# ur-whitelab/nmrgnn

Hardware: AMD Instinct MI355X
Metric: atoms/s (fwd+bwd) on 256-atom/16-neighbor synthetic graphs (higher is better)
Workload: dtype f32 (2xf16-piece MFMA, f32 accumulate)

## Files before the change

include/nmrgnn_hip.h:

```cpp
#ifndef NMRGNN_HIP_H
#define NMRGNN_HIP_H

#include <stdint.h>

#ifdef __cplusplus
extern "C" {
#endif

#define NG_ABI_VERSION 9

enum {
  NG_OK = 0,
  NG_ERR_INVALID = -1,
  NG_ERR_HIP = -2,
  NG_ERR_NOMEM = -3,
  NG_ERR_UNSUPPORTED = -4
};

enum { NG_ACT_NONE = 0, NG_ACT_SOFTPLUS = 1, NG_ACT_RELU = 2, NG_ACT_TANH = 3 };

typedef struct ng_ctx ng_ctx;

int ng_abi_version(void);
int ng_ctx_create(int device, ng_ctx** out);
void ng_ctx_destroy(ng_ctx* ctx);
const char* ng_last_error(ng_ctx* ctx);
int ng_reload_env(void);
int ng_weights_frozen(ng_ctx* ctx, int owner);
int ng_weights_changed(ng_ctx* ctx);
int ng_defer_reductions(ng_ctx* ctx, void* stream, int on);
int ng_flush_reductions(ng_ctx* ctx, void* stream);
int ng_ctx_set_graph_span(ng_ctx* ctx, int64_t max_graph_atoms);
int ng_ctx_reserve(ng_ctx* ctx, uint64_t bytes);

int ng_replay_arm(ng_ctx* ctx, int on);
int ng_replay_stage(ng_ctx* ctx, void* stream, uint64_t seed, float lr, float beta1, float beta2, int64_t step, int n_copies,
                    const void* const* src, void* const* dst, const uint64_t* bytes);
int ng_replay_token(ng_ctx* ctx, uint64_t* token);
int ng_replay_commit(ng_ctx* ctx, uint64_t token);

int ng_prof_enable(ng_ctx* ctx, int on);
int ng_prof_reset(ng_ctx* ctx);
int ng_prof_read(ng_ctx* ctx, int cap, const char** names, double* total_ms, int64_t* count);

int ng_randn(ng_ctx*, void* stream, uint64_t seed, uint64_t offset, float* out, int64_t n);
int ng_dropout_mask(ng_ctx*, void* stream, uint64_t seed, uint64_t offset, float keep, float* out,
                    int64_t n);

int ng_add_noise(ng_ctx*, void* stream, uint64_t seed, uint64_t offset, int64_t n, const float* x, float alpha,
                 float* out);
int ng_add_scaled(ng_ctx*, void* stream, int64_t n, const float* x, const float* y, float alpha,
                  float* out);

int ng_rbf_expand(ng_ctx*, void* stream, int64_t n, int H, const float* d_src, const float* d_eff,
                  const float* centers, float gap, float* out);

int ng_edge_mlp_fwd(ng_ctx*, void* stream, int64_t n_edges, int H, int E, int Le, int act,
                    const float* d_src, const float* d_eff, const float* centers, float gap,
                    const float* const* W, const float* const* b, float* e_out, float* z_save);
int ng_edge_tape_layout(int H, int E, int Le, int act, int64_t n_edges);
int ng_edge_mlp_bwd(ng_ctx*, void* stream, int64_t n_edges, int H, int E, int Le, int act,
                    const float* d_src, const float* d_eff, const float* centers, float gap,
                    const float* const* W, const float* z_save, const float* de,
                    float* const* dW, float* const* db);
int ng_edge_mlp_bwd_tape(ng_ctx*, void* stream, int64_t n_edges, int H, int E, int Le, int act,
                         const float* d_src, const float* d_eff, const float* centers, float gap,
                         const float* const* W, const float* z_save, const float* de,
                         float* const* dW, float* const* db, int tape_layout);

int ng_build_live_edges(ng_ctx*, void* stream, int64_t n_slots, const float* edges, int32_t* perm, int32_t* pos,
                        float* d_c, int32_t* n_live);
int ng_build_graph_lists(ng_ctx*, void* stream, int64_t N, int K, const int32_t* nlist, const float* edges, int32_t* nlist_c,
                         int32_t* csc_ptr, int32_t* csc_edge, int32_t* perm, int32_t* pos, float* d_c, int32_t* n_live);
int ng_graph_lists_one_launch(int64_t N, int K);
int ng_add_noise_live(ng_ctx*, void* stream, uint64_t seed, uint64_t offset, int64_t n, const float* x, const float* y,
                      float alpha, const int32_t* pos, float* out_c);
int ng_edge_live_supported(int H, int E, int Le, int act);
int ng_edge_mlp_fwd_live(ng_ctx*, void* stream, int64_t n_slots, int H, int E, int Le, int act,
                         const float* d_src_c, const float* d_eff_c, const int32_t* perm, const int32_t* n_live,
                         const float* centers, float gap, const float* const* W, const float* const* b,
                         float* e_out, float* z_save);
int ng_edge_mlp_bwd_live(ng_ctx*, void* stream, int64_t n_slots, int H, int E, int Le, int act,
                         const float* d_src_c, const float* d_eff_c, const int32_t* perm, const int32_t* n_live,
                         const float* centers, float gap, const float* const* W, const float* z_save,
                         const float* de, float* const* dW, float* const* db, int tape_layout);

int ng_edge_mlp_dinput(ng_ctx*, void* stream, int64_t n_slots, int H, int E, int Le, int act, const float* d_src,
                       const float* d_eff, const int32_t* perm, const int32_t* n_live, const float* centers, float gap,
                       const float* const* W, const float* const* b, const float* de, float* J_out, float* dd_out);
int ng_positions_grad(ng_ctx*, void* stream, int64_t N, int K, const float* pos, const int32_t* nlist, const float* edges,
                      const float* dd, float scale, const int32_t* csc_ptr, const int32_t* csc_edge, float* dpos);
int ng_positions_grad_csr(ng_ctx*, void* stream, int64_t N, int64_t nnz, const float* pos, const int32_t* row_ptr,
                          const int32_t* col, const int32_t* row_of, const float* dd, float scale, const int32_t* csc_ptr,
                          const int32_t* csc_edge, float* dpos);
int ng_positions_grad_pbc(ng_ctx*, void* stream, int64_t N, int K, const float* pos, const int32_t* nlist,
                          const float* edges, const float* dd, float scale, const int32_t* csc_ptr, const int32_t* csc_edge,
                          int n, const float* box, int triclinic, float* dpos);
int ng_positions_grad_csr_pbc(ng_ctx*, void* stream, int64_t N, int64_t nnz, const float* pos, const int32_t* row_ptr,
                              const int32_t* col, const int32_t* row_of, const float* dd, float scale,
                              const int32_t* csc_ptr, const int32_t* csc_edge, int n, const float* box, int triclinic,
                              float* dpos);
int ng_box_grad(ng_ctx*, void* stream, int64_t N, int K, const float* pos, const int32_t* nlist, const float* edges,
                const float* dd, float scale, int G, const int32_t* graph_ptr, const float* box, int triclinic, double* strain,
                double* dvec);
int ng_box_grad_csr(ng_ctx*, void* stream, int64_t N, int64_t nnz, const float* pos, const int32_t* row_ptr,
                    const int32_t* col, const float* dd, float scale, int G, const int32_t* graph_ptr, const float* box,
                    int triclinic, double* strain, double* dvec);
int ng_positions_grad_ragged_pbc(ng_ctx*, void* stream, int64_t N, int K, const float* pos, const int32_t* nlist,
                                 const float* edges, const float* dd, float scale, const int32_t* csc_ptr,
                                 const int32_t* csc_edge, int G, const int32_t* graph_ptr, const float* box,
                                 const int32_t* kind, const int32_t* kind_host, float* dpos);
int ng_positions_grad_csr_ragged_pbc(ng_ctx*, void* stream, int64_t N, int64_t nnz, const float* pos, const int32_t* row_ptr,
                                     const int32_t* col, const int32_t* row_of, const float* dd, float scale,
                                     const int32_t* csc_ptr, const int32_t* csc_edge, int G, const int32_t* graph_ptr,
                                     const float* box, const int32_t* kind, const int32_t* kind_host, float* dpos);
int ng_box_grad_ragged(ng_ctx*, void* stream, int64_t N, int K, const float* pos, const int32_t* nlist, const float* edges,
                       const float* dd, float scale, int G, const int32_t* graph_ptr, const float* box, const int32_t* kind,
                       const int32_t* kind_host, double* strain, double* dvec);
int ng_box_grad_csr_ragged(ng_ctx*, void* stream, int64_t N, int64_t nnz, const float* pos, const int32_t* row_ptr,
                           const int32_t* col, const float* dd, float scale, int G, const int32_t* graph_ptr,
                           const float* box, const int32_t* kind, const int32_t* kind_host, double* strain, double* dvec);

int ng_embed_fwd(ng_ctx*, void* stream, int64_t N, int C, int F, const float* atoms,
                 const float* Wemb, float* h0);
int ng_embed_bwd(ng_ctx*, void* stream, int64_t N, int C, int F, const float* atoms,
                 const float* dh0, float* dWemb);

int ng_mp_aggregate(ng_ctx*, void* stream, int64_t N, int K, int F, int E, const float* h,
                    const int32_t* nlist, const float* e, float* A);

int ng_mp_layer_fwd(ng_ctx*, void* stream, int64_t N, int K, int F, int E, int act, int residual,
                    const float* h, const int32_t* nlist, const float* e, const float* inv_degree,
                    const float* w, float* h_out, float* A_save, float* s_save);
int ng_mp_layer_wants_aggregate(int F, int E, int K);

int ng_mp_layer_bwd(ng_ctx*, void* stream, int64_t N, int K, int F, int E, int act,
                    const float* h, const int32_t* nlist, const float* e, const float* inv_degree,
                    const float* w, const float* A_save, const float* s_save,
                    const int32_t* csc_ptr, const int32_t* csc_edge, const float* dh_out,
                    float* dh_in, float* de, int de_accum, float* dw);

int ng_mp_edge_records(ng_ctx*, void* stream, int64_t N, int K, int E, const int32_t* csc_ptr,
                       const int32_t* csc_edge, const float* e, float* rec);
int ng_mp_layer_bwd_rec(ng_ctx*, void* stream, int64_t N, int K, int F, int E, int act,
                    const float* h, const int32_t* nlist, const float* e, const float* inv_degree,
                    const float* w, const float* A_save, const float* s_save,
                    const int32_t* csc_ptr, const int32_t* csc_edge, const float* dh_out,
                    float* dh_in, float* de, int de_accum, float* dw, const float* csc_rec);

int ng_mp_aggregate_csr(ng_ctx*, void* stream, int64_t N, int F, int E, const float* h,
                        const int32_t* row_ptr, const int32_t* col, const float* e, float* A);
int ng_mp_layer_fwd_csr(ng_ctx*, void* stream, int64_t N, int64_t nnz, int F, int E, int act, int residual,
                        const float* h, const int32_t* row_ptr, const int32_t* col, const float* e,
                        const float* inv_degree, const float* w, float* h_out, float* A_save, float* s_save);
int ng_mp_layer_bwd_csr(ng_ctx*, void* stream, int64_t N, int64_t nnz, int F, int E, int act, const float* h,
                        const int32_t* row_ptr, const int32_t* col, const int32_t* row_of, const float* e,
                        const float* inv_degree, const float* w, const float* A_save, const float* s_save,
                        const int32_t* csc_ptr, const int32_t* csc_edge, const float* dh_out, float* dh_in,
                        float* de, int de_accum, float* dw);

int ng_mp_layer_fwd_short(ng_ctx*, void* stream, int64_t N, int K, int F, int E, int act, int residual, const float* h,
                          const int32_t* nlist, const float* e, const float* inv_degree, const float* w, float* h_out);
int ng_mp_layer_fwd_short_csr(ng_ctx*, void* stream, int64_t N, int F, int E, int act, int residual, const float* h,
                              const int32_t* row_ptr, const int32_t* col, const float* e, const float* inv_degree,
                              const float* w, float* h_out);
int ng_mp_layer_short_ok(int64_t N, int K, int F, int E);
int ng_fc_head_ok(int64_t N, int F, int L, int C, int act);
int ng_fc_head_fwd(ng_ctx*, void* stream, int64_t N, int F, int L, int C, int act, const float* x,
                   const float* const* W, const float* const* b, const float* Wout, const float* bout,
                   const float* atoms, const float* pstd, const float* pavg, float* peaks);

int ng_build_incoming_lists(ng_ctx*, void* stream, int64_t N, int K, int64_t n_entries, const int32_t* nlist,
                            const float* edges, int32_t* nlist_c, int32_t* csc_ptr, int32_t* csc_edge);
size_t ng_incoming_lists_scratch_bytes(int64_t N, int64_t n_entries);

int ng_cutoff_count(ng_ctx*, void* stream, int G, int n, float cutoff, const float* pos, int32_t* deg);
int ng_cutoff_fill(ng_ctx*, void* stream, int G, int n, float cutoff, float scale, const float* pos,
                   const int32_t* row_ptr, int32_t* col, float* dist, float* inv_degree);
int ng_cutoff_fill_rows(ng_ctx*, void* stream, int G, int n, float cutoff, float scale, const float* pos,
                        const int32_t* row_ptr, int32_t* col, float* dist, float* inv_degree, int32_t* row_of);
int ng_cutoff_count_pbc(ng_ctx*, void* stream, int G, int n, float cutoff, const float* pos, const float* box, int triclinic,
                        int32_t* deg);
int ng_cutoff_fill_rows_pbc(ng_ctx*, void* stream, int G, int n, float cutoff, float scale, const float* pos,
                            const float* box, int triclinic, const int32_t* row_ptr, int32_t* col, float* dist,
                            float* inv_degree, int32_t* row_of);
int ng_exclusive_scan_i32(ng_ctx*, void* stream, int64_t n, const int32_t* in, int32_t* out);

int ng_knn_graph(ng_ctx*, void* stream, int G, int n, int K, float scale, const float* pos,
                 int32_t* nlist, float* edges, float* inv_degree);
int ng_knn_graph_pbc(ng_ctx*, void* stream, int G, int n, int K, float scale, const float* pos, const float* box,
                     int triclinic, int32_t* nlist, float* edges, float* inv_degree);
int ng_knn_graph_ragged(ng_ctx*, void* stream, int G, int64_t N, int K, float scale, const float* pos, const int32_t* graph_ptr,
                        const int32_t* graph_ptr_host, int max_n, int32_t* nlist, float* edges, float* inv_degree);
int ng_cutoff_count_ragged(ng_ctx*, void* stream, int G, int64_t N, float cutoff, const float* pos, const int32_t* graph_ptr,
                           int max_n, int32_t* deg);
int ng_cutoff_fill_rows_ragged(ng_ctx*, void* stream, int G, int64_t N, float cutoff, float scale, const float* pos,
                               const int32_t* graph_ptr, int max_n, const int32_t* row_ptr, int32_t* col, float* dist,
                               float* inv_degree, int32_t* row_of);
int ng_knn_graph_ragged_pbc(ng_ctx*, void* stream, int G, int64_t N, int K, float scale, const float* pos,
                            const int32_t* graph_ptr, const int32_t* graph_ptr_host, int max_n, const float* box,
                            const int32_t* kind, const int32_t* kind_host, int32_t* nlist, float* edges, float* inv_degree);
int ng_cutoff_count_ragged_pbc(ng_ctx*, void* stream, int G, int64_t N, float cutoff, const float* pos,
                               const int32_t* graph_ptr, int max_n, const float* box, const int32_t* kind,
                               const int32_t* kind_host, int32_t* deg);
int ng_cutoff_fill_rows_ragged_pbc(ng_ctx*, void* stream, int G, int64_t N, float cutoff, float scale, const float* pos,
                                   const int32_t* graph_ptr, int max_n, const float* box, const int32_t* kind,
                                   const int32_t* kind_host, const int32_t* row_ptr, int32_t* col, float* dist,
                                   float* inv_degree, int32_t* row_of);

int ng_amp_attend(ng_ctx*, void* stream, int64_t N, int K, int F, int E, const float* h,
                  const int32_t* nlist, const float* e, const float* inv_degree, const float* wq,
                  const float* wk, float* agg);
int ng_amp_attend_bwd(ng_ctx*, void* stream, int64_t N, int K, int F, int E, const float* h,
                      const int32_t* nlist, const float* e, const float* inv_degree, const float* wq,
                      const float* wk, const int32_t* in_ptr, const int32_t* in_slot, const float* dagg,
                      float* dh, float* de, float* dwq, float* dwk);

int ng_fc_block_fwd(ng_ctx*, void* stream, int64_t N, int F, int L, int act, const float* x,
                    const float* const* W, const float* const* b, float* const* y, float* g);

int64_t ng_fc_block_scratch_floats(int64_t N, int F, int L);
int ng_fc_block_bwd(ng_ctx*, void* stream, int64_t N, int F, int L, int act, const float* const* x,
                    const float* g, const float* const* W, const float* dg, float* dx, float* const* dW,
                    float* const* db, float* scratch);

int ng_dense_fwd(ng_ctx*, void* stream, int64_t M, int Kin, int Nout, int act, int residual,
                 const float* X, const float* W, const float* b, float* Y, float* s_save);
int ng_dense_bwd(ng_ctx*, void* stream, int64_t M, int Kin, int Nout, int act, int residual,
                 const float* X, const float* W, const float* s_save, const float* dY, float* dX,
                 float* dW, float* db);

// ... 64 lines not shown
```

nmrgnn_amd/_lib.py:

```python
from __future__ import annotations

import ctypes as C
import os
import threading

_HERE = os.path.dirname(os.path.abspath(__file__))
LIB_PATH = os.environ.get("NMRGNN_HIP_LIB") or os.path.join(_HERE, "csrc", "libnmrgnn_hip.so")

NG_ACT_NONE, NG_ACT_SOFTPLUS, NG_ACT_RELU, NG_ACT_TANH = 0, 1, 2, 3
ACT_CODES = {None: NG_ACT_NONE, "linear": NG_ACT_NONE, "softplus": NG_ACT_SOFTPLUS, "relu": NG_ACT_RELU,
             "tanh": NG_ACT_TANH}

_c_float_p = C.POINTER(C.c_float)
_c_int32_p = C.POINTER(C.c_int32)
_vp = C.c_void_p
_i64 = C.c_int64
_u64 = C.c_uint64
_int = C.c_int
_f = C.c_float

SIGNATURES = {
    "ng_abi_version": (_int, []),
    "ng_ctx_create": (_int, [_int, C.POINTER(_vp)]),
    "ng_ctx_destroy": (None, [_vp]),
    "ng_last_error": (C.c_char_p, [_vp]),
    "ng_ctx_reserve": (_int, [_vp, _u64]),
    "ng_replay_arm": (_int, [_vp, _int]),
    "ng_replay_stage": (_int, [_vp, _vp, _u64, _f, _f, _f, _i64, _int, C.POINTER(_vp), C.POINTER(_vp), C.POINTER(_u64)]),
    "ng_replay_token": (_int, [_vp, C.POINTER(_u64)]),
    "ng_replay_commit": (_int, [_vp, _u64]),
    "ng_reload_env": (_int, []),
    "ng_weights_frozen": (_int, [_vp, _int]),
    "ng_weights_changed": (_int, [_vp]),
    "ng_defer_reductions": (_int, [_vp, _vp, _int]),
    "ng_flush_reductions": (_int, [_vp, _vp]),
    "ng_ctx_set_graph_span": (_int, [_vp, _i64]),
    "ng_prof_enable": (_int, [_vp, _int]),
    "ng_prof_reset": (_int, [_vp]),
    "ng_prof_read": (_int, [_vp, _int, C.POINTER(C.c_char_p), C.POINTER(C.c_double), C.POINTER(_i64)]),
    "ng_randn": (_int, [_vp, _vp, _u64, _u64, _vp, _i64]),
    "ng_dropout_mask": (_int, [_vp, _vp, _u64, _u64, _f, _vp, _i64]),
    "ng_add_scaled": (_int, [_vp, _vp, _i64, _vp, _vp, _f, _vp]),
    "ng_add_noise": (_int, [_vp, _vp, _u64, _u64, _i64, _vp, _f, _vp]),
    "ng_rbf_expand": (_int, [_vp, _vp, _i64, _int, _vp, _vp, _vp, _f, _vp]),
    "ng_edge_mlp_fwd": (_int, [_vp, _vp, _i64, _int, _int, _int, _int, _vp, _vp, _vp, _f,
                               C.POINTER(_vp), C.POINTER(_vp), _vp, _vp]),
    "ng_edge_tape_layout": (_int, [_int, _int, _int, _int, _i64]),
    "ng_edge_table_range": (_int, [_vp, _vp, _i64, _int, _vp, _vp, _vp, _vp, _f, _vp]),
    "ng_edge_table_points": (_int, [_vp, _vp, _int, _int, _vp, _vp, _vp, _vp]),
    "ng_edge_table_check": (_int, [_vp, _vp, _int, _int, _vp, _f, _vp, _vp, _vp, _int, _vp, _vp]),
    "ng_edge_table_interp": (_int, [_vp, _vp, _i64, _int, _int, _vp, _vp, _vp, _vp, _vp, _vp, _vp]),
    "ng_edge_table_scatter": (_int, [_vp, _vp, _i64, _int, _int, _int, _vp, _vp, _vp, _vp, _vp, _vp]),
    "ng_edge_table_dinput": (_int, [_vp, _vp, _i64, _int, _int, _vp, _vp, _vp, _vp, _vp, _vp, _vp, _vp]),
    "ng_edge_mlp_bwd": (_int, [_vp, _vp, _i64, _int, _int, _int, _int, _vp, _vp, _vp, _f,
                               C.POINTER(_vp), _vp, _vp, C.POINTER(_vp), C.POINTER(_vp)]),
    "ng_edge_mlp_bwd_tape": (_int, [_vp, _vp, _i64, _int, _int, _int, _int, _vp, _vp, _vp, _f,
                                    C.POINTER(_vp), _vp, _vp, C.POINTER(_vp), C.POINTER(_vp), _int]),
    "ng_build_live_edges": (_int, [_vp, _vp, _i64, _vp, _vp, _vp, _vp, _vp]),
    "ng_build_graph_lists": (_int, [_vp, _vp, _i64, _int, _vp, _vp, _vp, _vp, _vp, _vp, _vp, _vp, _vp]),
    "ng_graph_lists_one_launch": (_int, [_i64, _int]),
    "ng_add_noise_live": (_int, [_vp, _vp, _u64, _u64, _i64, _vp, _vp, _f, _vp, _vp]),
    "ng_edge_live_supported": (_int, [_int, _int, _int, _int]),
    "ng_edge_mlp_fwd_live": (_int, [_vp, _vp, _i64, _int, _int, _int, _int, _vp, _vp, _vp, _vp, _vp, _f,
                                    C.POINTER(_vp), C.POINTER(_vp), _vp, _vp]),
    "ng_edge_mlp_bwd_live": (_int, [_vp, _vp, _i64, _int, _int, _int, _int, _vp, _vp, _vp, _vp, _vp, _f,
                                    C.POINTER(_vp), _vp, _vp, C.POINTER(_vp), C.POINTER(_vp), _int]),
    "ng_edge_mlp_dinput": (_int, [_vp, _vp, _i64, _int, _int, _int, _int, _vp, _vp, _vp, _vp, _vp, _f,
                                  C.POINTER(_vp), C.POINTER(_vp), _vp, _vp, _vp]),
    "ng_positions_grad": (_int, [_vp, _vp, _i64, _int, _vp, _vp, _vp, _vp, _f, _vp, _vp, _vp]),
    "ng_positions_grad_csr": (_int, [_vp, _vp, _i64, _i64, _vp, _vp, _vp, _vp, _vp, _f, _vp, _vp, _vp]),
    "ng_positions_grad_pbc": (_int, [_vp, _vp, _i64, _int, _vp, _vp, _vp, _vp, _f, _vp, _vp, _int, _vp, _int, _vp]),
    "ng_positions_grad_csr_pbc": (_int, [_vp, _vp, _i64, _i64, _vp, _vp, _vp, _vp, _vp, _f, _vp, _vp, _int, _vp, _int, _vp]),
    "ng_box_grad": (_int, [_vp, _vp, _i64, _int, _vp, _vp, _vp, _vp, _f, _int, _vp, _vp, _int, _vp, _vp]),
    "ng_box_grad_csr": (_int, [_vp, _vp, _i64, _i64, _vp, _vp, _vp, _vp, _f, _int, _vp, _vp, _int, _vp, _vp]),
    "ng_positions_grad_ragged_pbc": (_int, [_vp, _vp, _i64, _int, _vp, _vp, _vp, _vp, _f, _vp, _vp, _int, _vp, _vp, _vp, _vp, _vp]),
    "ng_positions_grad_csr_ragged_pbc": (_int, [_vp, _vp, _i64, _i64, _vp, _vp, _vp, _vp, _vp, _f, _vp, _vp, _int, _vp, _vp, _vp,
                                                _vp, _vp]),
    "ng_box_grad_ragged": (_int, [_vp, _vp, _i64, _int, _vp, _vp, _vp, _vp, _f, _int, _vp, _vp, _vp, _vp, _vp, _vp]),
    "ng_box_grad_csr_ragged": (_int, [_vp, _vp, _i64, _i64, _vp, _vp, _vp, _vp, _f, _int, _vp, _vp, _vp, _vp, _vp, _vp]),
    "ng_restraint_loss": (_int, [_vp, _vp, _int, _i64, _vp, _vp, _vp, _vp, _vp]),
    "ng_restraint_loss_ex": (_int, [_vp, _vp, _int, _i64, _int, _vp, _vp, _vp, _vp, _vp, _f, _vp, _vp, _vp, _vp]),
    "ng_embed_fwd": (_int, [_vp, _vp, _i64, _int, _int, _vp, _vp, _vp]),
    "ng_embed_bwd": (_int, [_vp, _vp, _i64, _int, _int, _vp, _vp, _vp]),
    "ng_mp_aggregate": (_int, [_vp, _vp, _i64, _int, _int, _int, _vp, _vp, _vp, _vp]),
    "ng_mp_layer_fwd": (_int, [_vp, _vp, _i64, _int, _int, _int, _int, _int, _vp, _vp, _vp, _vp, _vp,
                               _vp, _vp, _vp]),
    "ng_mp_layer_bwd": (_int, [_vp, _vp, _i64, _int, _int, _int, _int, _vp, _vp, _vp, _vp, _vp,
                               _vp, _vp, _vp, _vp, _vp, _vp, _vp, _int, _vp]),
    "ng_mp_layer_bwd_rec": (_int, [_vp, _vp, _i64, _int, _int, _int, _int, _vp, _vp, _vp, _vp, _vp,
                               _vp, _vp, _vp, _vp, _vp, _vp, _vp, _int, _vp, _vp]),
    "ng_mp_edge_records": (_int, [_vp, _vp, _i64, _int, _int, _vp, _vp, _vp, _vp]),
    "ng_mp_aggregate_csr": (_int, [_vp, _vp, _i64, _int, _int, _vp, _vp, _vp, _vp, _vp]),
    "ng_mp_layer_fwd_csr": (_int, [_vp, _vp, _i64, _i64, _int, _int, _int, _int, _vp, _vp, _vp, _vp, _vp, _vp,
                                   _vp, _vp, _vp]),
    "ng_mp_layer_bwd_csr": (_int, [_vp, _vp, _i64, _i64, _int, _int, _int, _vp, _vp, _vp, _vp, _vp, _vp, _vp,
                                   _vp, _vp, _vp, _vp, _vp, _vp, _vp, _int, _vp]),
    "ng_build_incoming_lists": (_int, [_vp, _vp, _i64, _int, _i64, _vp, _vp, _vp, _vp, _vp]),
    "ng_incoming_lists_scratch_bytes": (C.c_size_t, [_i64, _i64]),
    "ng_cutoff_count": (_int, [_vp, _vp, _int, _int, _f, _vp, _vp]),
    "ng_cutoff_fill": (_int, [_vp, _vp, _int, _int, _f, _f, _vp, _vp, _vp, _vp, _vp]),
    "ng_cutoff_fill_rows": (_int, [_vp, _vp, _int, _int, _f, _f, _vp, _vp, _vp, _vp, _vp, _vp]),
    "ng_cutoff_count_pbc": (_int, [_vp, _vp, _int, _int, _f, _vp, _vp, _int, _vp]),
    "ng_cutoff_fill_rows_pbc": (_int, [_vp, _vp, _int, _int, _f, _f, _vp, _vp, _int, _vp, _vp, _vp, _vp, _vp]),
    "ng_exclusive_scan_i32": (_int, [_vp, _vp, _i64, _vp, _vp]),
    "ng_dense_fwd": (_int, [_vp, _vp, _i64, _int, _int, _int, _int, _vp, _vp, _vp, _vp, _vp]),
    "ng_dense_bwd": (_int, [_vp, _vp, _i64, _int, _int, _int, _int, _vp, _vp, _vp, _vp, _vp, _vp,
                            _vp]),
    "ng_head_fwd": (_int, [_vp, _vp, _i64, _int, _int, _vp, _vp, _vp, _vp, _vp, _vp, _vp, _vp]),
    "ng_head_fwd_dropout": (_int, [_vp, _vp, _i64, _int, _int, _vp, _u64, _u64, _f, _vp, _vp, _vp, _vp, _vp, _vp, _vp]),
    "ng_head_bwd": (_int, [_vp, _vp, _i64, _int, _int, _vp, _vp, _vp, _vp, _vp, _vp, _vp, _vp, _vp]),
    "ng_head_loss_blocks": (_int, [_vp, _int, _int, _int, _i64]),
    "ng_head_loss_bwd": (_int, [_vp, _vp, _i64, _int, _int, _int, _i64, _vp, _u64, _u64, _f, _vp, _vp, _vp, _vp, _vp, _vp, _vp,
                               _vp, _vp, _f, _vp, _vp, _vp]),
    "ng_head_loss_reduce": (_int, [_vp, _vp, _vp, _int, _int, _int, _vp, _vp, _vp]),
    "ng_mp_layer_wants_aggregate": (_int, [_int, _int, _int]),
    "ng_fc_block_fwd": (_int, [_vp, _vp, _i64, _int, _int, _int, _vp, _vp, _vp, _vp, _vp]),
    "ng_fc_block_scratch_floats": (_i64, [_i64, _int, _int]),
    "ng_fc_block_bwd": (_int, [_vp, _vp, _i64, _int, _int, _int, _vp, _vp, _vp, _vp, _vp, _vp, _vp, _vp]),
    "ng_mp_layer_fwd_short": (_int, [_vp, _vp, _i64, _int, _int, _int, _int, _int, _vp, _vp, _vp, _vp, _vp, _vp]),
    "ng_mp_layer_fwd_short_csr": (_int, [_vp, _vp, _i64, _int, _int, _int, _int, _vp, _vp, _vp, _vp, _vp, _vp, _vp]),
    "ng_mp_layer_short_ok": (_int, [_i64, _int, _int, _int]),
    "ng_fc_head_ok": (_int, [_i64, _int, _int, _int, _int]),
    "ng_fc_head_fwd": (_int, [_vp, _vp, _i64, _int, _int, _int, _int, _vp, C.POINTER(_vp), C.POINTER(_vp), _vp, _vp, _vp,
                              _vp, _vp, _vp]),
    "ng_knn_graph": (_int, [_vp, _vp, _int, _int, _int, _f, _vp, _vp, _vp, _vp]),
    "ng_knn_graph_pbc": (_int, [_vp, _vp, _int, _int, _int, _f, _vp, _vp, _int, _vp, _vp, _vp]),
    "ng_knn_graph_ragged": (_int, [_vp, _vp, _int, _i64, _int, _f, _vp, _vp, _vp, _int, _vp, _vp, _vp]),
    "ng_cutoff_count_ragged": (_int, [_vp, _vp, _int, _i64, _f, _vp, _vp, _int, _vp]),
    "ng_cutoff_fill_rows_ragged": (_int, [_vp, _vp, _int, _i64, _f, _f, _vp, _vp, _int, _vp, _vp, _vp, _vp, _vp]),
    "ng_knn_graph_ragged_pbc": (_int, [_vp, _vp, _int, _i64, _int, _f, _vp, _vp, _vp, _int, _vp, _vp, _vp, _vp, _vp, _vp]),
    "ng_cutoff_count_ragged_pbc": (_int, [_vp, _vp, _int, _i64, _f, _vp, _vp, _int, _vp, _vp, _vp, _vp]),
    "ng_cutoff_fill_rows_ragged_pbc": (_int, [_vp, _vp, _int, _i64, _f, _f, _vp, _vp, _int, _vp, _vp, _vp, _vp, _vp, _vp, _vp,
                                              _vp]),
    "ng_amp_attend": (_int, [_vp, _vp, _i64, _int, _int, _int, _vp, _vp, _vp, _vp, _vp, _vp, _vp]),
    "ng_amp_attend_bwd": (_int, [_vp, _vp, _i64, _int, _int, _int] + [_vp] * 13),
    "ng_loss_l2": (_int, [_vp, _vp, _i64, _int, _vp, _vp, _vp, _vp, _vp, _vp]),
    "ng_loss_name": (_int, [_vp, _vp, _i64, _int, _vp, _vp, _vp, _vp, _f, _vp, _vp]),
    "ng_name_metrics": (_int, [_vp, _vp, _i64, _vp, _vp, _vp, _vp, _int, _vp, _int, _int, _vp]),
    "ng_adam_step": (_int, [_vp, _vp, _i64, _vp, _vp, _vp, _vp, _f, _f, _f, _f, _i64, _f]),
    "ng_comm_unique_id": (_int, [_vp]),
    "ng_comm_init": (_int, [_vp, _int, _int, _vp]),
    "ng_comm_destroy": (_int, [_vp]),
    "ng_comm_world": (_int, [_vp]),
    "ng_allreduce_grads": (_int, [_vp, _vp, _vp, _i64]),
}

_lib = None
_lock = threading.Lock()


class NGError(RuntimeError):
    pass


def load():
    global _lib
    with _lock:
        if _lib is not None:
            return _lib
        if not os.path.exists(LIB_PATH):
            raise NGError(
                f"{LIB_PATH} is missing — build it with `python -c 'import __graft_entry__ as g; "
                f"g.build()'` or `make -C nmrgnn_amd/csrc`. nmrgnn_amd has no CPU fallback.")
        lib = C.CDLL(LIB_PATH)
        for name, (res, args) in SIGNATURES.items():
            fn = getattr(lib, name)
            fn.restype = res
            fn.argtypes = args
        if lib.ng_abi_version() != 9:
            raise NGError("libnmrgnn_hip.so ABI version mismatch")
        _lib = lib
        return lib

# ... 73 lines not shown
```

nmrgnn_amd/csrc/edge_bwd_h2.hip:

```cpp
#include "edge_bwd_h2.cuh"

namespace ng {

template <bool LIVE>
__global__ __launch_bounds__(HX_THREADS, 1) void edge_bwd_h2_kernel(EdgeBwdH2Args a) {
  extern __shared__ __attribute__((aligned(16))) char smem_hx[];
  float* sWo4 = reinterpret_cast<float*>(smem_hx + HX_IMGS);
  float* sdE = sWo4 + FH * 4;
  float* sCen = sdE + FTM * 4;

  const int tid = threadIdx.x, lane = tid & 63, half = lane >> 5, l31 = lane & 31;
  const int wave = __builtin_amdgcn_readfirstlane(tid >> 6);
  const int kslab = wave >> 1, nsl0 = 2 * (wave & 1);
  const int zk = wave & 3, zrt = wave >> 2;
  const int cn = tid & 127, rq = tid >> 7;
  const int row = 32 * zrt + l31;
  const int col0 = 32 * zk + 4 * half;
  const int prz = hx_prow_z(row), prg = hx_prow_g(row);
  const int E = a.E;
  if (LIVE && __builtin_amdgcn_readfirstlane(*a.n_live) < 0) return;
  float gscale, ginv;
  {
    float* sred = reinterpret_cast<float*>(smem_hx);
    float m = 0.f;
// ... 236 lines not shown
    for (int r = 0; r < 16; ++r) chk += fabsf(accB[r]);
#pragma unroll
    for (int n = 0; n < 4; ++n) chk += fabsf(accWo[n]) + fabsf(accbo[n]);
    range_guard_raise(a.guard, not_finite(chk * ginv));
  }
  {
    const int k = kslab * 32 + l31;
#pragma unroll
    for (int l = 0; l < 3; ++l)
#pragma unroll
      for (int j = 0; j < 2; ++j)
#pragma unroll
        for (int q = 0; q < 4; ++q) {
          const int n = (nsl0 + j) * 32 + 8 * q + 4 * half;
          *reinterpret_cast<float4*>(part + l * FH * FH + k * FH + n) =
              make_float4(ginv * accW[l][j][4 * q + 0], ginv * accW[l][j][4 * q + 1], ginv * accW[l][j][4 * q + 2],
                          ginv * accW[l][j][4 * q + 3]);
        }
  }
  float* red = reinterpret_cast<float*>(smem_hx);
  float* dbw = reinterpret_cast<float*>(smem_hx + 2 * HX_IMG_Z);
  const int red_stride = 3 * FH + FH * E + E;
  {
    const int c = l31 / 5;
    if (c < 6 && l31 == 5 * c && (c & 1) >= 0) {
      const int layer = c >> 1, j = c & 1;
#pragma unroll
      for (int r = 0; r < 16; ++r)
        dbw[(kslab * 3 + layer) * FH + 32 * (nsl0 + j) + (r & 3) + 8 * (r >> 2) + 4 * half] = ginv * accB[r];
    }
  }
  if (zk == 0 && half == 0) *reinterpret_cast<float4*>(sdE + 4 * row) = make_float4(accbo[0], accbo[1], accbo[2], accbo[3]);
  __syncthreads();
#pragma unroll
  for (int l = 0; l < 3; ++l) red[rq * red_stride + l * FH + cn] = dbw[(rq * 3 + l) * FH + cn];
  for (int n = 0; n < E; ++n) red[rq * red_stride + 3 * FH + cn * E + n] = ginv * accWo[n];
  if (cn < E) {
    float sbo = 0.f;
    if (rq == 0)
      for (int r = 0; r < FTM; ++r) sbo += sdE[4 * r + cn];
    red[rq * red_stride + 3 * FH + FH * E + cn] = ginv * sbo;
  }
  __syncthreads();
  for (int t = tid; t < red_stride; t += HX_THREADS)
    part[3 * FH * FH + t] = red[t] + red[red_stride + t] + red[2 * red_stride + t] + red[3 * red_stride + t];
}

constexpr int HX_SCALE_BLOCKS = 1024;
constexpr int64_t HX_DIRECT_MAX = 32768;
__global__ __launch_bounds__(256) void hx_absmax_kernel(const float* __restrict__ de, int64_t n, float* __restrict__ blockmax,
                                                        const int32_t* __restrict__ n_live) {
  __shared__ float red[4];
  if (n_live && *n_live < 0) return;
  float m = 0.f;
  const int64_t n4 = (reinterpret_cast<uintptr_t>(de) & 15) == 0 ? n >> 2 : 0;
  const float4* de4 = reinterpret_cast<const float4*>(de);
  for (int64_t i = (int64_t)blockIdx.x * 256 + threadIdx.x; i < n4; i += (int64_t)gridDim.x * 256) {
    const float4 v = de4[i];
    m = fmaxf(fmaxf(m, fmaxf(fabsf(v.x), fabsf(v.y))), fmaxf(fabsf(v.z), fabsf(v.w)));
  }
  for (int64_t i = 4 * n4 + (int64_t)blockIdx.x * 256 + threadIdx.x; i < n; i += (int64_t)gridDim.x * 256) m = fmaxf(m, fabsf(de[i]));
#pragma unroll
  for (int o = 32; o > 0; o >>= 1) m = fmaxf(m, __shfl_xor(m, o));
  if ((threadIdx.x & 63) == 0) red[threadIdx.x >> 6] = m;
  __syncthreads();
  if (threadIdx.x == 0) blockmax[blockIdx.x] = fmaxf(fmaxf(red[0], red[1]), fmaxf(red[2], red[3]));
}

constexpr int64_t HX_SEG_EDGES = ((int64_t)1 << 23) - 256;
int edge_bwd_h2_segments(int64_t n_edges) { return (int)std::max<int64_t>(1, cdiv(n_edges, HX_SEG_EDGES)); }

bool edge_bwd_h2_supported(int E, int64_t n_edges) { (void)n_edges; return E >= 1 && E <= 4; }

bool edge_tape_blocked(int E, int64_t n_edges) {
  return edge_split_enabled() && !sw().edge_bwd_math_fp32 && edge_bwd_h2_supported(E, n_edges);
}
constexpr size_t HX_WT_BYTES = (size_t)2 * 4 * 8 * 2 * 1024;

size_t edge_bwd_h2_ws_bytes() { return HX_WT_BYTES + 16 + (size_t)(HX_SCALE_BLOCKS + 2) * 4; }

int edge_bwd_h2_launch(ng_ctx* ctx, hipStream_t st, int64_t n_edges, int E, const float* d_src, const float* d_eff,
                       const float* centers, float gap, const float* const* W, const float* z_save, const float* de,
                       char* wt_img, float* partial, int part_stride, int grid, int tape_blocked, RangeGuard guard,
                       LiveEdges live) {
  float* blockmax = reinterpret_cast<float*>(wt_img + HX_WT_BYTES + 16);
  int nb_max = 0;
  bool have_wt = false;
  char* wimg = (char*)cached_image(ctx, W[1], 13, HX_WT_BYTES + 16, &have_wt);
  const bool cached_wt = wimg != nullptr;
  if (!wimg) wimg = wt_img;
  {
    ProfScope ps(ctx, st, "edge_bwd_h2_prep");
    if (!have_wt) {
      PackJob j;
      j.kind = PK_EDGE_WT; j.blocks = 17; j.src[0] = W[1]; j.src[1] = W[2]; j.src[2] = W[3]; j.i0 = E; j.dst[0] = wimg;
      if (int rc = pack_launch(ctx, st, j)) return rc;
      if (cached_wt) cache_set_job(ctx, W[1], 13, j);
    }
    if (n_edges * E <= HX_DIRECT_MAX && (reinterpret_cast<uintptr_t>(de) & 15) == 0) {
      nb_max = -(int)(n_edges * E);
      blockmax = const_cast<float*>(de);
    } else {
      nb_max = (int)std::min<int64_t>(HX_SCALE_BLOCKS, cdiv(n_edges * E, 1024));
      hipLaunchKernelGGL(hx_absmax_kernel, dim3(nb_max), dim3(256), 0, st, de, n_edges * E, blockmax, live.n_live);
      NG_HIP(ctx, hipGetLastError());
    }
  }
  const int nseg = edge_bwd_h2_segments(n_edges);
  for (int sg = 0; sg < nseg; ++sg) {
    const int64_t e0 = (int64_t)sg * HX_SEG_EDGES;
    EdgeBwdH2Args a;
    a.n_edges = std::min<int64_t>(HX_SEG_EDGES, n_edges - e0); a.d_src = d_src + e0; a.d_eff = d_eff + e0; a.centers = centers;
    a.neg_inv_gap_log2e = (float)(-1.4426950408889634 / (double)gap);
    a.wt_img = wimg; a.blockmax = blockmax; a.n_blockmax = nb_max; a.Wo = W[3]; a.z_save = z_save + e0 * FH; a.z_layer_stride = n_edges * FH;
    a.de = live.perm ? de : de + e0 * E;
    a.perm = live.perm ? live.perm + e0 : nullptr; a.n_live = live.n_live; a.row_base = e0;
    a.partial = partial + (size_t)sg * grid * part_stride; a.part_stride = part_stride; a.E = E; a.tape_blocked = tape_blocked;
    a.guard = guard;
    ProfScope ps(ctx, st, "edge_bwd_h2");
    if (live.perm)
      hipLaunchKernelGGL(edge_bwd_h2_kernel<true>, dim3(grid), dim3(HX_THREADS), HX_LDS_BYTES, st, a);
    else
      hipLaunchKernelGGL(edge_bwd_h2_kernel<false>, dim3(grid), dim3(HX_THREADS), HX_LDS_BYTES, st, a);
    NG_HIP(ctx, hipGetLastError());
    if (sg + 1 < nseg) continue;
  }
  return NG_OK;
}

}
```

nmrgnn_amd/csrc/edge_fused.h:

```cpp
#pragma once
#include "ng_internal.h"

namespace ng {

constexpr int FH = 128;
constexpr int FTM = 64;
constexpr int FLD = FH + 4;
constexpr int FMAX_E = 8;

int edge_fused_pack(ng_ctx* ctx, hipStream_t st, const float* const* W, float* Wpk, float* WpkT);
PackJob edge_fused_pack_job(const float* const* W, float* Wpk, float* WpkT);

}

namespace ng {
int edge_fused_bwd(ng_ctx* ctx, hipStream_t st, int64_t n_edges, int E, const float* d_src,
                   const float* d_eff, const float* centers, float gap, const float* const* W,
                   const float* z_save, const float* de, float* const* dW, float* const* db, int tape_layout = -1,
                   LiveEdges live = LiveEdges());
}

#define NG_LDS_BARRIER()                                   \
  do {                                                     \
    asm volatile("s_waitcnt lgkmcnt(0)" ::: "memory");     \
    __builtin_amdgcn_s_barrier();                          \
    asm volatile("" ::: "memory");                         \
  } while (0)

namespace ng {
bool edge_split_enabled();
int edge_h2_fwd(ng_ctx* ctx, hipStream_t st, int64_t n_edges, int E, const float* d_src, const float* d_eff,
                const float* centers, float gap, const float* const* W, const float* const* b, float* e_out,
                float* z_save, LiveEdges live = LiveEdges());
bool edge_bwd_h2_supported(int E, int64_t n_edges);
int edge_bwd_h2_segments(int64_t n_edges);
bool edge_tape_blocked(int E, int64_t n_edges);
size_t edge_bwd_h2_ws_bytes();
int edge_bwd_h2_launch(ng_ctx* ctx, hipStream_t st, int64_t n_edges, int E, const float* d_src, const float* d_eff,
                       const float* centers, float gap, const float* const* W, const float* z_save, const float* de,
                       char* wt_img, float* partial, int part_stride, int grid, int tape_blocked, RangeGuard guard,
                       LiveEdges live = LiveEdges());
}
```

nmrgnn_amd/csrc/edge_fused_bwd.hip:

```cpp
#include <algorithm>

#include "mfma_gemm.cuh"
#include "edge_fused.h"

namespace ng {

constexpr int BW_THREADS = 512;

struct EdgeBwdArgs {
  int64_t n_edges;
  const float* d_src;
  const float* d_eff;
  const float* centers;
  float neg_inv_gap;
  const float* WpkT;
  const float* Wo;
  const float* z_save;
  const float* de;
  float* partial;
  int part_stride;
  int tape_blocked;
  int zero_rows;
  RangeGuard guard;
  const int32_t* perm;
// ... 209 lines not shown
      o.z = g[2] * (1.0f - __expf(-z.z));
      o.w = g[3] * (1.0f - __expf(-z.w));
      *reinterpret_cast<float4*>(bufC + row * FLD + c4 * 4) = o;
    }
#pragma unroll 4
    for (int r = 16 * rq; r < 16 * rq + 16; ++r) {
      const float z = bufA[r * FLD + cn];
#pragma unroll
      for (int n = 0; n < E; ++n) accWo[n] += z * sdE[r * E + n];
      if (cn < E) accbo += sdE[r * E + cn];
    }
    regs_to_lds(pzB, bufB, tid);
    NG_LDS_BARRIER();
    dw_gemm(accW[2], bufB, bufC, kslab, nsl0, lane);
    colsum16(accb[2], bufC, cn, rq);
    dz_gemm_epilogue(bufC, bufB, bufA, a.WpkT, 2, zk, zrt, lane);
    NG_LDS_BARRIER();
    regs_to_lds(pzA, bufC, tid);
    NG_LDS_BARRIER();
    dw_gemm(accW[1], bufC, bufA, kslab, nsl0, lane);
    colsum16(accb[1], bufA, cn, rq);
    dz_gemm_epilogue(bufA, bufC, bufB, a.WpkT, 1, zk, zrt, lane);
    NG_LDS_BARRIER();
#pragma unroll
    for (int i = 0; i < 4; ++i) {
      const int lin = tid + i * BW_THREADS;
      const int row = lin >> 5, c4 = lin & 31;
      const float d = sD[row], m = sM[row];
      const float4 mu = *reinterpret_cast<const float4*>(sCen + c4 * 4);
      const float u0 = d - mu.x, u1 = d - mu.y, u2 = d - mu.z, u3 = d - mu.w;
      float4 o;
      o.x = m * __expf(u0 * u0 * a.neg_inv_gap);
      o.y = m * __expf(u1 * u1 * a.neg_inv_gap);
      o.z = m * __expf(u2 * u2 * a.neg_inv_gap);
      o.w = m * __expf(u3 * u3 * a.neg_inv_gap);
      *reinterpret_cast<float4*>(bufA + row * FLD + c4 * 4) = o;
    }
    NG_LDS_BARRIER();
    if (tile + gridDim.x < ntiles) prefetch((tile + gridDim.x) * FTM);
    dw_gemm(accW[0], bufA, bufB, kslab, nsl0, lane);
    colsum16(accb[0], bufB, cn, rq);
    NG_LDS_BARRIER();
  }

  float* part = a.partial + (int64_t)blockIdx.x * a.part_stride;
  {
    const int half = lane >> 5, l31 = lane & 31;
    const int k = kslab * 32 + l31;
#pragma unroll
    for (int l = 0; l < 3; ++l)
#pragma unroll
      for (int j = 0; j < 2; ++j)
#pragma unroll
        for (int q = 0; q < 4; ++q) {
          const int n = (nsl0 + j) * 32 + 8 * q + 4 * half;
          *reinterpret_cast<float4*>(part + l * FH * FH + k * FH + n) =
              make_float4(accW[l][j][4 * q + 0], accW[l][j][4 * q + 1], accW[l][j][4 * q + 2],
                          accW[l][j][4 * q + 3]);
        }
  }
  float* red = bufA;
  const int red_stride = 3 * FH + FH * E + E;
#pragma unroll
  for (int l = 0; l < 3; ++l) red[rq * red_stride + l * FH + cn] = accb[l];
#pragma unroll
  for (int n = 0; n < E; ++n) red[rq * red_stride + 3 * FH + cn * E + n] = accWo[n];
  if (cn < E) red[rq * red_stride + 3 * FH + FH * E + cn] = accbo;
  __syncthreads();
  for (int t = tid; t < red_stride; t += BW_THREADS)
    part[3 * FH * FH + t] = red[t] + red[red_stride + t] + red[2 * red_stride + t] + red[3 * red_stride + t];
  for (int64_t rowz = (int64_t)gridDim.x + blockIdx.x; rowz < a.zero_rows; rowz += gridDim.x)
    for (int t = tid; t < a.part_stride; t += BW_THREADS) a.partial[rowz * a.part_stride + t] = 0.f;
}

struct BwdOut {
  float* dW[3];
  float* db[3];
  float* dWo;
  float* dbo;
};

__global__ __launch_bounds__(1024) void edge_bwd_reduce_kernel(const float* __restrict__ partial, int n_wg,
                                                               int stride, int E, BwdOut o, const int32_t* __restrict__ n_live) {
  __shared__ float red[16][64];
  const int total = bwd_part_floats(E);
  const int lane = threadIdx.x & 63, wv = threadIdx.x >> 6;
  const int idx = blockIdx.x * 64 + lane;
  float s = 0.f;
  if (n_live && *n_live < 0) n_wg = 0;
  if (idx < total) {
    const float* p = partial + idx;
    int w = wv;
    for (; w + 112 < n_wg; w += 128) {
      float v[8];
#pragma unroll
      for (int u = 0; u < 8; ++u) v[u] = p[(int64_t)(w + 16 * u) * stride];
#pragma unroll
      for (int u = 0; u < 8; ++u) s += v[u];
    }
    for (; w < n_wg; w += 16) s += p[(int64_t)w * stride];
  }
  red[wv][lane] = s;
  __syncthreads();
  if (wv != 0 || idx >= total) return;
  s = red[0][lane];
#pragma unroll
  for (int j = 1; j < 16; ++j) s += red[j][lane];
  int r = idx;
  if (r < 3 * FH * FH) { o.dW[r / (FH * FH)][r % (FH * FH)] = s; return; }
  r -= 3 * FH * FH;
  if (r < 3 * FH) { o.db[r / FH][r % FH] = s; return; }
  r -= 3 * FH;
  if (r < FH * E) { o.dWo[r] = s; return; }
  r -= FH * E;
  o.dbo[r] = s;
}

int edge_fused_bwd(ng_ctx* ctx, hipStream_t st, int64_t n_edges, int E, const float* d_src,
                   const float* d_eff, const float* centers, float gap, const float* const* W,
                   const float* z_save, const float* de, float* const* dW, float* const* db, int tape_layout,
                   LiveEdges live) {
  const int64_t ntiles = cdiv(n_edges, FTM);
  const int grid = (int)std::min<int64_t>(ntiles, (int64_t)ctx->num_cu);
  const int stride = (bwd_part_floats(E) + 3) / 4 * 4;
  const size_t pk_floats = (size_t)3 * FH * FH;
  const int nseg = edge_bwd_h2_segments(n_edges);
  bool haveT = false;
  float* WpkT = (float*)cached_image(ctx, W[0], 12, pk_floats * 4, &haveT);
  const bool cachedT = WpkT != nullptr;
  float* ws = (float*)workspace(ctx, (pk_floats + (size_t)nseg * grid * stride) * 4 + edge_bwd_h2_ws_bytes());
  if (!ws) return NG_ERR_NOMEM;
  if (!cachedT) WpkT = ws;
  float* partial = ws + pk_floats;
  if (!haveT) {
    const PackJob j = edge_fused_pack_job(W, nullptr, WpkT);
    if (int rc = pack_launch(ctx, st, j)) return rc;
    if (cachedT) cache_set_job(ctx, W[0], 12, j);
  }
  EdgeBwdArgs a;
  a.n_edges = n_edges; a.d_src = d_src; a.d_eff = d_eff; a.centers = centers;
  a.neg_inv_gap = (float)(-1.0 / (double)gap);
  a.WpkT = WpkT; a.Wo = W[3]; a.z_save = z_save; a.de = de;
  a.partial = partial; a.part_stride = stride;
  a.tape_blocked = 0; a.zero_rows = 0; a.guard = RangeGuard{nullptr, 0};
  a.perm = live.perm; a.n_live = live.n_live; a.z_layer_stride = n_edges * FH;
  const size_t lds = (size_t)(3 * FTM * FLD + FH * FMAX_E + FTM * FMAX_E + 2 * FTM + FH) * 4;
  const bool blocked = tape_layout < 0 ? edge_tape_blocked(E, n_edges) : tape_layout == 1;
  if (blocked && !edge_bwd_h2_supported(E, n_edges)) return fail(ctx, NG_ERR_INVALID, "edge_mlp_bwd: blocked tape for an unsupported shape");
  int n_part = grid;
  const bool split = blocked || edge_tape_blocked(E, n_edges);
  if (split) {
    const RangeGuard guard = range_guard_begin(ctx);
    if (!guard.word) return NG_ERR_NOMEM;
    int rc3 = edge_bwd_h2_launch(ctx, st, n_edges, E, d_src, d_eff, centers, gap, W, z_save, de,
                     (char*)(partial + (size_t)nseg * grid * stride), partial, stride, grid, blocked ? 1 : 0, guard, live);
    if (rc3) return rc3;
    n_part = nseg * grid;
    a.tape_blocked = blocked ? 1 : 0; a.zero_rows = n_part; a.guard = guard;
  }
  {
    ProfScope ps(ctx, st, split ? "edge_bwd_range_fallback" : "edge_fused_bwd");
#define NG_BW(EE)                                                                                   \
  case EE:                                                                                          \
    hipLaunchKernelGGL((edge_fused_bwd_kernel<EE>), dim3(grid), dim3(BW_THREADS), lds, st, a);      \
    break;
    switch (E) { NG_BW(1) NG_BW(2) NG_BW(3) NG_BW(4) NG_BW(5) NG_BW(6) NG_BW(7) NG_BW(8) }
#undef NG_BW
    NG_HIP(ctx, hipGetLastError());
  }
  {
    ProfScope ps(ctx, st, "edge_bwd_reduce");
    BwdOut o;
    for (int l = 0; l < 3; ++l) { o.dW[l] = dW[l]; o.db[l] = db[l]; }
    o.dWo = dW[3]; o.dbo = db[3];
    hipLaunchKernelGGL(edge_bwd_reduce_kernel, dim3((unsigned)cdiv(bwd_part_floats(E), 64)), dim3(1024), 0, st,
                       partial, n_part, stride, E, o, live.n_live);
    NG_HIP(ctx, hipGetLastError());
  }
  return NG_OK;
}

}
```

nmrgnn_amd/csrc/edge_ops.hip:

```cpp
#include <algorithm>

#include "mfma_gemm.cuh"
#include "edge_fused.h"

namespace ng {

constexpr int MAX_E = 8;

__global__ void rbf_kernel(int64_t n_edges, int H, const float* __restrict__ d_src,
                           const float* __restrict__ d_eff, const float* __restrict__ centers,
                           float neg_inv_gap, float* __restrict__ X0) {
  const int c4n = H / 4;
  const int64_t total = n_edges * c4n;
  for (int64_t t = (int64_t)blockIdx.x * blockDim.x + threadIdx.x; t < total;
       t += (int64_t)gridDim.x * blockDim.x) {
    const int64_t eidx = t / c4n;
    const int c4 = (int)(t % c4n);
    float4 v = f4zero();
    if (d_src[eidx] > 0.f) {
      const float d = d_eff[eidx];
      const float4 mu = *reinterpret_cast<const float4*>(centers + c4 * 4);
      const float a = d - mu.x, b = d - mu.y, c = d - mu.z, dd = d - mu.w;
      v.x = __expf(a * a * neg_inv_gap);
      v.y = __expf(b * b * neg_inv_gap);
// ... 263 lines not shown
      rc = dense_dx(ctx, st, n_edges, H, H, act, dz, s_t, nullptr, W[t], nullptr, dz_next,
                    "edge_dense_dx");
      if (rc) return rc;
      std::swap(dz, dz_next);
    }
  }
  return NG_OK;
}

static bool force_layered() {
  return sw().edge_layered;
}

}

using namespace ng;

extern "C" int ng_rbf_expand(ng_ctx* ctx, void* stream, int64_t n, int H, const float* d_src,
                             const float* d_eff, const float* centers, float gap, float* out) {
  if (!ctx) return NG_ERR_INVALID;
  NG_REQUIRE(ctx, H % 4 == 0 && gap > 0.f, "rbf_expand: H % 4 == 0, gap > 0");
  if (n == 0) return NG_OK;
  ProfScope ps(ctx, (hipStream_t)stream, "rbf");
  hipLaunchKernelGGL(rbf_kernel, ew_grid(n * (H / 4)), dim3(256), 0, (hipStream_t)stream, n, H, d_src,
                     d_eff, centers, (float)(-1.0 / (double)gap), out);
  NG_HIP(ctx, hipGetLastError());
  return NG_OK;
}

static bool use_fused(int H, int E, int Le, int act) {
  return act == NG_ACT_SOFTPLUS && edge_fused_supported(H, E, Le) && !force_layered();
}

static int check_edge_shape(ng_ctx* ctx, int H, int E, int Le, int act) {
  NG_REQUIRE(ctx, H % 16 == 0 && H <= 512, "edge_mlp: edge_hidden_size % 16 == 0, <= 512");
  NG_REQUIRE(ctx, E >= 1 && (E <= MAX_E || (E % 4 == 0 && E <= 256)), "edge_mlp: edge_feature_size <= 8, or a multiple of 4 up to 256");
  NG_REQUIRE(ctx, Le >= 2, "edge_mlp: edge_fc_layers >= 2");
  NG_REQUIRE(ctx, act == NG_ACT_SOFTPLUS || act == NG_ACT_RELU || act == NG_ACT_TANH || act == NG_ACT_NONE,
             "edge_mlp: unknown activation code");
  return NG_OK;
}

extern "C" int ng_edge_mlp_fwd(ng_ctx* ctx, void* stream, int64_t n_edges, int H, int E, int Le, int act,
                               const float* d_src, const float* d_eff, const float* centers,
                               float gap, const float* const* W, const float* const* b,
                               float* e_out, float* z_save) {
  if (!ctx) return NG_ERR_INVALID;
  if (int rc = check_edge_shape(ctx, H, E, Le, act)) return rc;
  NG_REQUIRE(ctx, gap > 0.f, "edge_mlp: rbf gap > 0");
  if (n_edges == 0) return NG_OK;
  if (use_fused(H, E, Le, act))
    return edge_fused_fwd(ctx, (hipStream_t)stream, n_edges, E, d_src, d_eff, centers, gap, W, b,
                          e_out, z_save);
  return edge_mlp_fwd_layered(ctx, (hipStream_t)stream, n_edges, H, E, Le, act, d_src, d_eff, centers,
                              gap, W, b, e_out, z_save);
}

extern "C" int ng_edge_live_supported(int H, int E, int Le, int act) { return use_fused(H, E, Le, act) ? 1 : 0; }

static int check_live(ng_ctx* ctx, int64_t n_slots, int H, int E, int Le, int act, const int32_t* perm, const int32_t* n_live) {
  NG_REQUIRE(ctx, perm && n_live, "edge_mlp live view: perm and n_live required");
  NG_REQUIRE(ctx, use_fused(H, E, Le, act), "edge_mlp live view: only the fused edge path has it (ng_edge_live_supported)");
  NG_REQUIRE(ctx, n_slots > 0 && n_slots * (int64_t)E * 4 < ((int64_t)1 << 31), "edge_mlp live view: n_slots * E * 4 must stay below 2^31");
  return NG_OK;
}

extern "C" int ng_edge_mlp_fwd_live(ng_ctx* ctx, void* stream, int64_t n_slots, int H, int E, int Le, int act,
                                    const float* d_src_c, const float* d_eff_c, const int32_t* perm, const int32_t* n_live,
                                    const float* centers, float gap, const float* const* W, const float* const* b,
                                    float* e_out, float* z_save) {
  if (!ctx) return NG_ERR_INVALID;
  if (int rc = check_edge_shape(ctx, H, E, Le, act)) return rc;
  NG_REQUIRE(ctx, gap > 0.f, "edge_mlp: rbf gap > 0");
  if (n_slots == 0) return NG_OK;
  if (int rc = check_live(ctx, n_slots, H, E, Le, act, perm, n_live)) return rc;
  return edge_fused_fwd(ctx, (hipStream_t)stream, n_slots, E, d_src_c, d_eff_c, centers, gap, W, b, e_out, z_save,
                        LiveEdges{perm, n_live});
}

extern "C" int ng_edge_mlp_bwd_live(ng_ctx* ctx, void* stream, int64_t n_slots, int H, int E, int Le, int act,
                                    const float* d_src_c, const float* d_eff_c, const int32_t* perm, const int32_t* n_live,
                                    const float* centers, float gap, const float* const* W, const float* z_save,
                                    const float* de, float* const* dW, float* const* db, int tape_layout) {
  if (!ctx) return NG_ERR_INVALID;
  if (int rc = check_edge_shape(ctx, H, E, Le, act)) return rc;
  NG_REQUIRE(ctx, z_save, "edge_mlp_bwd: saved activations required");
  NG_REQUIRE(ctx, n_slots > 0, "edge_mlp_bwd live view: n_slots > 0");
  if (int rc = check_live(ctx, n_slots, H, E, Le, act, perm, n_live)) return rc;
  return edge_fused_bwd(ctx, (hipStream_t)stream, n_slots, E, d_src_c, d_eff_c, centers, gap, W, z_save, de, dW, db,
                        tape_layout, LiveEdges{perm, n_live});
}

extern "C" int ng_edge_tape_layout(int H, int E, int Le, int act, int64_t n_edges) {
  return use_fused(H, E, Le, act) && edge_tape_blocked(E, n_edges) ? 1 : 0;
}

extern "C" int ng_edge_mlp_bwd_tape(ng_ctx* ctx, void* stream, int64_t n_edges, int H, int E, int Le, int act,
                                    const float* d_src, const float* d_eff, const float* centers,
                                    float gap, const float* const* W, const float* z_save,
                                    const float* de, float* const* dW, float* const* db, int tape_layout) {
  if (!ctx) return NG_ERR_INVALID;
  if (int rc = check_edge_shape(ctx, H, E, Le, act)) return rc;
  NG_REQUIRE(ctx, z_save, "edge_mlp_bwd: saved activations required");
  hipStream_t st = (hipStream_t)stream;
  if (n_edges == 0) {
    for (int t = 0; t < Le; ++t) {
      const int kout = t < Le - 1 ? H : E;
      NG_HIP(ctx, hipMemsetAsync(dW[t], 0, (size_t)H * kout * 4, st));
      NG_HIP(ctx, hipMemsetAsync(db[t], 0, (size_t)kout * 4, st));
    }
    return NG_OK;
  }
  if (use_fused(H, E, Le, act))
    return edge_fused_bwd(ctx, st, n_edges, E, d_src, d_eff, centers, gap, W, z_save, de, dW, db, tape_layout);
  NG_REQUIRE(ctx, tape_layout != 1, "edge_mlp_bwd: a blocked tape needs the fused edge path");
  return edge_mlp_bwd_layered(ctx, st, n_edges, H, E, Le, act, d_src, d_eff, centers, gap, W, z_save, de,
                              dW, db);
}

extern "C" int ng_edge_mlp_bwd(ng_ctx* ctx, void* stream, int64_t n_edges, int H, int E, int Le, int act,
                               const float* d_src, const float* d_eff, const float* centers,
                               float gap, const float* const* W, const float* z_save,
                               const float* de, float* const* dW, float* const* db) {
  return ng_edge_mlp_bwd_tape(ctx, stream, n_edges, H, E, Le, act, d_src, d_eff, centers, gap, W, z_save, de, dW, db, -1);
}
```

nmrgnn_amd/csrc/mp_win16_bwd.hip:

```cpp
#include <algorithm>

#include "mfma_gemm.cuh"
#include "ng_internal.h"
#include "edge_fused.h"
#include "h2_common.cuh"
#include "mp_win_common.cuh"

namespace ng {
namespace w16b {

using namespace w16c;

constexpr int PROWB = (WF + 8) * 2, PPLANE = WTA * PROWB;
constexpr int SDP_LD = 68;
constexpr int DP_BYTES = 2 * PPLANE;
static_assert(DP_BYTES >= WTA * SDP_LD * 4, "the dP slot holds either form");

struct Args {
  int64_t N;
  int K;
  int64_t ntiles;
  int tiles_per_wg;
  const float* dH;
  const float* S;
  const float* rowscale;
  const float* h;
  const int32_t* nlist;
  const float* WfragT;
  const float* WfragT32;
  float* dP;
  float* de;
  float* dummy;
  int act;
  int accumulate;
  RangeGuard guard;
  const unsigned* wflag;
  unsigned wflag_ver;
};

template <int E, bool H2, int ACT = -1>
__device__ __forceinline__ void body(const Args& a) {
  const int act_ = ACT >= 0 ? ACT : a.act;
  constexpr int KF = E * WF;
  constexpr int LD = KF + 4;
  constexpr int NCT = KF / 16;
  extern __shared__ __attribute__((aligned(16))) float smem[];
  float* win = smem;
  float* tile = win + WROWS * WF;
  char* planes = reinterpret_cast<char*>(tile + WTA * LD);
  float* s_inv = reinterpret_cast<float*>(planes + DP_BYTES);
  int* ctl = reinterpret_cast<int*>(s_inv + WTA);

  const int tid = threadIdx.x, lane = tid & 63;
  const int wave = __builtin_amdgcn_readfirstlane(tid >> 6);
  const int K = a.K;
  const int64_t T0 = (int64_t)blockIdx.x * a.tiles_per_wg;
  const int64_t T1 = std::min<int64_t>(T0 + a.tiles_per_wg, a.ntiles);
  if (T0 >= T1) return;

  const float4* src4 = reinterpret_cast<const float4*>(a.h);
  float4* win4 = reinterpret_cast<float4*>(win);
  for (int t = tid; t < WROWS * WC4; t += WTHREADS) win4[t] = f4zero();

  const bool mx = wave < NCT;
  const int a16 = lane & 15, g4 = lane >> 4;
  u32x4 wh[2], wl[2];
  if (H2 && mx) {
    const u32x4* p = reinterpret_cast<const u32x4*>(a.WfragT) + (size_t)(wave * 2) * 2 * 64 + lane;
#pragma unroll
    for (int Ts = 0; Ts < 2; ++Ts) { wh[Ts] = p[(2 * Ts) * 64]; wl[Ts] = p[(2 * Ts + 1) * 64]; }
#pragma unroll
    for (int Ts = 0; Ts < 2; ++Ts)
#pragma unroll
      for (int j = 0; j < 4; ++j) { asm volatile("" : "+v"(wh[Ts][j])); asm volatile("" : "+v"(wl[Ts][j])); }
  }

  const int al = wave * 4 + (lane >> 4);
  const int prow = tid >> 4, pc = tid & 15;
  int p_idx;
  float4 p_dh, p_s;
  float p_rs;
  float p_de[E];
  auto issue = [&](int64_t t) {
    const int64_t row = t * WTA + prow;
    const int64_t rc = row < a.N ? row : a.N - 1;
    p_idx = a.nlist[rc * K + (pc < K ? pc : 0)];
    p_dh = *reinterpret_cast<const float4*>(a.dH + rc * WF + 4 * pc);
    p_s = a.S ? *reinterpret_cast<const float4*>(a.S + rc * WF + 4 * pc) : f4zero();
    p_rs = a.rowscale[rc];
    if (row >= a.N) p_dh = f4zero();
  };
  auto issue_de = [&](int64_t t) {
    const int64_t row = t * WTA + prow;
    const int64_t rc = row < a.N ? row : a.N - 1;
    const int sc = pc < K ? pc : 0;
#pragma unroll
    for (int n = 0; n < E; ++n) p_de[n] = a.accumulate ? a.de[(rc * K + sc) * E + n] : 0.f;
  };
  auto commit = [&](int64_t t) {
    float4 g = p_dh;
    if (act_ != NG_ACT_NONE) {
      g.x *= act_grad_from_out(act_, p_s.x); g.y *= act_grad_from_out(act_, p_s.y);
      g.z *= act_grad_from_out(act_, p_s.z); g.w *= act_grad_from_out(act_, p_s.w);
    }
    g.x *= p_rs; g.y *= p_rs; g.z *= p_rs; g.w *= p_rs;
    if (H2) {
      float m = fmaxf(fmaxf(fabsf(g.x), fabsf(g.y)), fmaxf(fabsf(g.z), fabsf(g.w)));
      m = fmaxf(m, ror_f<8>(m)); m = fmaxf(m, ror_f<4>(m)); m = fmaxf(m, ror_f<2>(m)); m = fmaxf(m, ror_f<1>(m));
      const int ef = (__builtin_bit_cast(int, m) >> 23) & 255;
      const int sb = (ef == 0 || ef == 255) ? 127 : min(267 - ef, 253);
      const float S = __builtin_bit_cast(float, sb << 23);
      if (pc == 0) s_inv[prow] = __builtin_bit_cast(float, (254 - sb) << 23) * (1.0f / 256.0f);
      unsigned h0, l0, h1, l1;
      split2_pair(S * g.x, S * g.y, h0, l0); split2_pair(S * g.z, S * g.w, h1, l1);
      char* q = planes + prow * PROWB + 8 * pc;
      *reinterpret_cast<u32x2*>(q) = u32x2{h0, h1};
      *reinterpret_cast<u32x2*>(q + PPLANE) = u32x2{l0, l1};
    } else {
      *reinterpret_cast<float4*>(reinterpret_cast<float*>(planes) + prow * SDP_LD + 4 * pc) = g;
    }
    const int64_t row = t * WTA + prow;
    *reinterpret_cast<float4*>(row < a.N ? a.dP + row * WF + 4 * pc : a.dummy + 4 * pc) = g;
    const bool live = pc < K && row < a.N;
    int lo = live ? p_idx : 0x7fffffff, hi = live ? p_idx : -1;
    lo = wave_min_i32(lo);
    hi = -wave_min_i32(-hi);
    if (lane == 63) { ctl[(t & 1) * (2 * NW) + wave] = lo; ctl[(t & 1) * (2 * NW) + NW + wave] = hi; }
  };

  int wlo = -(1 << 30), mode = 0;
  issue(T0);
  commit(T0);
  int idx_cur = p_idx;
  issue(T0 + 1 < T1 ? T0 + 1 : T0);
  issue_de(T0);
  NG_LDS_BARRIER();

#pragma unroll 1
  for (int64_t t = T0; t < T1; ++t) {
    const bool staged = win_decide(ctl + (t & 1) * (2 * NW), wlo, mode);
    if (staged) win_dma(win, a.h, wlo, a.N, wave, lane);
    if (mx) {
      if (H2) {
#pragma unroll
        for (int rt = 0; rt < 4; ++rt) {
          const int r = 16 * rt + a16;
          const char* xr = planes + r * PROWB + 16 * g4;
          const u32x4 xh0 = *reinterpret_cast<const u32x4*>(xr), xl0 = *reinterpret_cast<const u32x4*>(xr + PPLANE);
          const u32x4 xh1 = *reinterpret_cast<const u32x4*>(xr + 64), xl1 = *reinterpret_cast<const u32x4*>(xr + 64 + PPLANE);
          f32x4 acc = {0.f, 0.f, 0.f, 0.f};
          acc = __builtin_amdgcn_mfma_f32_16x16x32_f16(__builtin_bit_cast(f16x8, wl[0]), __builtin_bit_cast(f16x8, xh0), acc, 0, 0, 0);
          acc = __builtin_amdgcn_mfma_f32_16x16x32_f16(__builtin_bit_cast(f16x8, wh[0]), __builtin_bit_cast(f16x8, xl0), acc, 0, 0, 0);
          acc = __builtin_amdgcn_mfma_f32_16x16x32_f16(__builtin_bit_cast(f16x8, wh[0]), __builtin_bit_cast(f16x8, xh0), acc, 0, 0, 0);
          acc = __builtin_amdgcn_mfma_f32_16x16x32_f16(__builtin_bit_cast(f16x8, wl[1]), __builtin_bit_cast(f16x8, xh1), acc, 0, 0, 0);
          acc = __builtin_amdgcn_mfma_f32_16x16x32_f16(__builtin_bit_cast(f16x8, wh[1]), __builtin_bit_cast(f16x8, xl1), acc, 0, 0, 0);
          acc = __builtin_amdgcn_mfma_f32_16x16x32_f16(__builtin_bit_cast(f16x8, wh[1]), __builtin_bit_cast(f16x8, xh1), acc, 0, 0, 0);
          const float osc = s_inv[r];
          *reinterpret_cast<float4*>(tile + r * LD + 16 * wave + 4 * g4) = make_float4(acc[0] * osc, acc[1] * osc, acc[2] * osc, acc[3] * osc);
        }
      } else {
        const float4* p32 = reinterpret_cast<const float4*>(a.WfragT32) + (size_t)(wave * 4) * 64 + lane;
#pragma unroll 1
        for (int rt = 0; rt < 4; ++rt) {
          const int r = 16 * rt + a16;
          const float* xrow = reinterpret_cast<const float*>(planes) + r * SDP_LD + 4 * g4;
          f32x4 acc = {0.f, 0.f, 0.f, 0.f};
#pragma unroll
          for (int T = 0; T < 4; ++T) {
            const float4 wv = p32[T * 64];
            const float4 x = *reinterpret_cast<const float4*>(xrow + 16 * T);
            acc = __builtin_amdgcn_mfma_f32_16x16x4f32(wv.x, x.x, acc, 0, 0, 0);
            acc = __builtin_amdgcn_mfma_f32_16x16x4f32(wv.y, x.y, acc, 0, 0, 0);
            acc = __builtin_amdgcn_mfma_f32_16x16x4f32(wv.z, x.z, acc, 0, 0, 0);
            acc = __builtin_amdgcn_mfma_f32_16x16x4f32(wv.w, x.w, acc, 0, 0, 0);
          }
          *reinterpret_cast<float4*>(tile + r * LD + 16 * wave + 4 * g4) = make_float4(acc[0], acc[1], acc[2], acc[3]);
        }
      }
    }
    if (staged) asm volatile("s_waitcnt vmcnt(0)" ::: "memory");
    NG_LDS_BARRIER();
    {
      float out[E];
      if (mode == 0) edge_dot<E, false>(lane, al, wlo, idx_cur, tile, LD, win4, src4, out);
      else {
        const EdgeDots<E> r = edge_dot_global<E>(lane, al, idx_cur, tile, LD, src4);
#pragma unroll
        for (int n = 0; n < E; ++n) out[n] = r.v[n];
      }
      const int64_t row = t * WTA + prow;
      const bool live = row < a.N && pc < K;
      float* dst = live ? a.de + (row * K + pc) * E : a.dummy;
#pragma unroll
      for (int n = 0; n < E; ++n) dst[n] = out[n] + p_de[n];
    }
    if (t + 1 < T1) commit(t + 1);
    idx_cur = p_idx;
    issue(t + 2 < T1 ? t + 2 : t);
    issue_de(t + 1 < T1 ? t + 1 : t);
    NG_LDS_BARRIER();
  }
}

template <int E>
__global__ __launch_bounds__(WTHREADS) void mp_win16_bwd_edge_kernel(Args a) {
  if (a.guard.word && (range_guard_raised(a.guard) || wimage_flag_raised(a.wflag))) body<E, false>(a);
  else if (a.act == NG_ACT_SOFTPLUS) body<E, true, NG_ACT_SOFTPLUS>(a);
  else body<E, true>(a);
}

}

static size_t mp_win16_bwd_edge_lds(int E) {
  return (size_t)(w16b::WROWS * w16b::WF + w16b::WTA * (E * w16b::WF + 4) + w16b::WTA + 4 * w16b::NW) * 4 + w16b::DP_BYTES;
}

bool mp_win16_bwd_edge_supported(int E, int K) { return E >= 1 && E <= 3 && K >= 1 && K <= 16; }

int mp_win16_bwd_edge_launch(ng_ctx* ctx, hipStream_t st, int64_t N, int K, int E, int act, const float* h, const int32_t* nlist,
                             const float* inv_degree, const float* WfragT, const float* s_save, const float* dh_out, float* dP,
                             float* de, int de_accum, float* dummy, RangeGuard guard, const float* WfragT32, const unsigned* wflag,
                             unsigned wflag_ver) {
  using namespace w16b;
  Args a{};
  a.N = N; a.K = K; a.ntiles = cdiv(N, WTA);
  const int64_t per = win_tiles_per_wg(a.ntiles, ctx->num_cu, 4);
  a.tiles_per_wg = (int)per;
  a.dH = dh_out; a.S = act == NG_ACT_NONE ? nullptr : s_save; a.rowscale = inv_degree; a.h = h;
  a.nlist = nlist; a.WfragT = WfragT; a.WfragT32 = WfragT32; a.dP = dP; a.de = de; a.dummy = dummy; a.act = act;
  a.accumulate = de_accum; a.guard = guard; a.wflag = wflag; a.wflag_ver = wflag_ver;
  const int grid = (int)cdiv(a.ntiles, per);
  const size_t lds = mp_win16_bwd_edge_lds(E);
  ProfScope ps(ctx, st, "mp_win_bwd_edge");
  switch (E) {
    case 1: hipLaunchKernelGGL((mp_win16_bwd_edge_kernel<1>), dim3(grid), dim3(WTHREADS), lds, st, a); break;
    case 2: hipLaunchKernelGGL((mp_win16_bwd_edge_kernel<2>), dim3(grid), dim3(WTHREADS), lds, st, a); break;
    case 3: hipLaunchKernelGGL((mp_win16_bwd_edge_kernel<3>), dim3(grid), dim3(WTHREADS), lds, st, a); break;
  }
  NG_HIP(ctx, hipGetLastError());
  return NG_OK;
}

}
```

nmrgnn_amd/csrc/mp_win_bwd.hip:

```cpp
#include <algorithm>
#include <cstdlib>
#include <cstring>

#include "mfma_gemm.cuh"
#include "ng_internal.h"
#include "edge_fused.h"
#include "reduce.cuh"
#include "h2_common.cuh"
#include "pack_bodies.cuh"
#include "mp_win_common.cuh"

namespace ng {

namespace {

using namespace w8c;

constexpr int SDP_LD = 68;
constexpr int SDP_SLOT = 2304;

typedef short gs16x4 __attribute__((ext_vector_type(4)));

__device__ __forceinline__ void win_dma(float* __restrict__ win, dma_i4 rs, int wlo, int wave, int lane) {
#pragma unroll
// ... 608 lines not shown
          const int sba = s_sb[at];
          const float ratio = sba < sbref ? 1.0f : __builtin_bit_cast(float, max(sbref - sba + 127, 0) << 23);
          hv[tt] = htile[at * SDP_LD + 16 * ct + a16] * ratio;
        }
        float hm = fmaxf(fmaxf(fmaxf(fabsf(hv[0]), fabsf(hv[1])), fmaxf(fabsf(hv[2]), fabsf(hv[3]))),
                         fmaxf(fmaxf(fabsf(hv[4]), fabsf(hv[5])), fmaxf(fabsf(hv[6]), fabsf(hv[7]))));
        f32x4 osc4 = {inv_ref, inv_ref, inv_ref, inv_ref};
        if (__builtin_amdgcn_ballot_w64(hm >= 32768.0f) != 0) {
          hm = fmaxf(hm, __shfl_xor(hm, 16));
          hm = fmaxf(hm, __shfl_xor(hm, 32));
          const int hef = (__builtin_bit_cast(int, hm) >> 23) & 255;
          const bool hbig = hef >= 127 + 15 && hef != 255;
          const float hs = hbig ? __builtin_bit_cast(float, (268 - hef) << 23) : 1.0f;
          const float hsi = hbig ? __builtin_bit_cast(float, (hef - 14) << 23) : 1.0f;
#pragma unroll
          for (int tt = 0; tt < 8; ++tt) hv[tt] *= hs;
#pragma unroll
          for (int r = 0; r < 4; ++r) osc4[r] = __shfl(hsi, 4 * g4 + r) * inv_ref;
        }
        unsigned h0, l0, h1, l1, h2, l2, h3, l3;
        split2_pair(hv[0], hv[1], h0, l0); split2_pair(hv[2], hv[3], h1, l1);
        split2_pair(hv[4], hv[5], h2, l2); split2_pair(hv[6], hv[7], h3, l3);
        const u32x4 ah = {h0, h1, h2, h3}, al = {l0, l1, l2, l3};
        const char* bp = planes + (8 * g4 + (a16 >> 2)) * ROWB + (16 * (NCT * hh) + 4 * (a16 & 3)) * 2;
#pragma unroll
        for (int u = 0; u < NCT; ++u) {
          const char* q0 = bp + 32 * u;
          const gs16x4 v0 = __builtin_amdgcn_ds_read_tr16_b64_v4i16((__attribute__((address_space(3))) gs16x4*)q0);
          const gs16x4 v1 = __builtin_amdgcn_ds_read_tr16_b64_v4i16((__attribute__((address_space(3))) gs16x4*)(q0 + 4 * ROWB));
          const gs16x4 w0 = __builtin_amdgcn_ds_read_tr16_b64_v4i16((__attribute__((address_space(3))) gs16x4*)(q0 + PLANE));
          const gs16x4 w1 = __builtin_amdgcn_ds_read_tr16_b64_v4i16((__attribute__((address_space(3))) gs16x4*)(q0 + PLANE + 4 * ROWB));
          const u32x2 a0 = __builtin_bit_cast(u32x2, v0), a1 = __builtin_bit_cast(u32x2, v1);
          const u32x2 c0 = __builtin_bit_cast(u32x2, w0), c1 = __builtin_bit_cast(u32x2, w1);
          const u32x4 bh = {a0[0], a0[1], a1[0], a1[1]}, bl = {c0[0], c0[1], c1[0], c1[1]};
          f32x4 at = {0.f, 0.f, 0.f, 0.f};
          at = __builtin_amdgcn_mfma_f32_16x16x32_f16(__builtin_bit_cast(f16x8, al), __builtin_bit_cast(f16x8, bh), at, 0, 0, 0);
          at = __builtin_amdgcn_mfma_f32_16x16x32_f16(__builtin_bit_cast(f16x8, ah), __builtin_bit_cast(f16x8, bl), at, 0, 0, 0);
          at = __builtin_amdgcn_mfma_f32_16x16x32_f16(__builtin_bit_cast(f16x8, ah), __builtin_bit_cast(f16x8, bh), at, 0, 0, 0);
          accW[u] += at * osc4;
        }
      } else if (DW) {
        const float* ha = htile + 16 * ct + a16;
        const float* bb = tile + 16 * (NCT * hh) + a16;
#pragma unroll
        for (int T = 0; T < 8; ++T) {
          const int ro = (T & 3) + 4 * g4 + 16 * (T >> 2);
          const float av = ha[ro * SDP_LD];
#pragma unroll
          for (int u = 0; u < NCT; ++u)
            accW[u] = __builtin_amdgcn_mfma_f32_16x16x4f32(av, bb[ro * LD + 16 * u], accW[u], 0, 0, 0);
        }
      }
      if (restage && dma_ok) asm volatile("s_waitcnt vmcnt(0)" ::: "memory");
      NG_LDS_BARRIER();
    }
  }
  if (DW) {
    float* part = a.partial + (int64_t)blockIdx.x * (KF * WF);
    const int a16 = lane & 15, g4 = lane >> 4;
#pragma unroll
    for (int u = 0; u < NCT; ++u) {
      const int cidx = 16 * (NCT * hh + u) + a16;
      *reinterpret_cast<float4*>(part + cidx * WF + 16 * ct + 4 * g4) =
          make_float4(accW[u][0], accW[u][1], accW[u][2], accW[u][3]);
    }
  }
}

template <int E, bool H2, bool DW>
__global__ __launch_bounds__(WTHREADS, 1) void mp_win_bwd_node_kernel(MpWinNodeArgs a) {
  if (H2 && a.guard.word && (range_guard_raised(a.guard) || wimage_flag_raised(a.wflag))) {
    a.WfragN = a.WfragN32;
    mp_win_bwd_node_body<E, false, DW>(a);
  } else {
    mp_win_bwd_node_body<E, H2, DW>(a);
  }
}

__global__ void mp_records_kernel(int64_t N, int K, int E, const int32_t* __restrict__ csc_ptr,
                                  const int32_t* __restrict__ csc_edge, const float* __restrict__ e,
                                  float4* __restrict__ rec, const int32_t* __restrict__ row_of) {
  const int64_t nnz = csc_ptr[N];
  const int64_t stride = (int64_t)gridDim.x * blockDim.x;
  for (int64_t p0 = (int64_t)blockIdx.x * blockDim.x + threadIdx.x; p0 < nnz; p0 += 4 * stride) {
    int eid[4];
#pragma unroll
    for (int u = 0; u < 4; ++u) eid[u] = csc_edge[std::min<int64_t>(p0 + u * stride, nnz - 1)];
    float4 r[4];
#pragma unroll
    for (int u = 0; u < 4; ++u) {
      r[u].x = __builtin_bit_cast(float, row_of ? row_of[eid[u]] : eid[u] / K);
      if (E == 3) {
        struct __attribute__((packed, aligned(4))) F3 { float x, y, z; };
        const F3 v = *reinterpret_cast<const F3*>(e + (int64_t)eid[u] * 3);
        r[u].y = v.x; r[u].z = v.y; r[u].w = v.z;
      } else {
        r[u].y = e[(int64_t)eid[u] * E];
        r[u].z = E > 1 ? e[(int64_t)eid[u] * E + 1] : 0.f;
        r[u].w = 0.f;
      }
    }
#pragma unroll
    for (int u = 0; u < 4; ++u)
      if (p0 + u * stride < nnz) rec[p0 + u * stride] = r[u];
  }
}

size_t node_lds_bytes(int E, bool h2) {
  return (size_t)(WROWS * WF + WTA * (E * WF + 4) + WTA * SDP_LD) * 4 + (size_t)2 * NREC_CAP * 16 + (2 * 36 + 32 + 32 + 32 + 8) * 4 +
         (h2 ? (size_t)2 * WTA * (E * WF + 8) * 2 : 0);
}

size_t edge_lds_bytes(int K, int E) {
  return (size_t)(WROWS * WF + WTA * (E * WF + 4) + 2 * SDP_SLOT + 2 * WTA * K + 32 + 2 * WTA) * 4;
}

}

static bool mp_win_bwd_h2() { return !sw().gemm_math_fp32; }

int mp_win_records(ng_ctx* ctx, hipStream_t st, int64_t N, int K, int E, const int32_t* csc_ptr,
                   const int32_t* csc_edge, const float* e, float* rec, const int32_t* row_of, int64_t n_entries) {
  if (N == 0) return NG_OK;
  ProfScope ps(ctx, st, "mp_records");
  const int grid = (int)std::min<int64_t>(cdiv(std::max<int64_t>(row_of ? n_entries : N * K, 1), 256), (int64_t)ctx->num_cu * 8);
  hipLaunchKernelGGL(mp_records_kernel, dim3(grid), dim3(256), 0, st, N, K, E, csc_ptr, csc_edge, e,
                     reinterpret_cast<float4*>(rec), row_of);
  NG_HIP(ctx, hipGetLastError());
  return NG_OK;
}

size_t mp_win_node_scratch_floats(ng_ctx* ctx, int E) { return (size_t)(ctx->num_cu + 1) * E * WF * WF; }

int mp_win_bwd_node(ng_ctx* ctx, hipStream_t st, int64_t N, int E, const float* h, const float* dP,
                    const int32_t* csc_ptr, const float* rec, const float* WfragN, const float* dh_out,
                    float* dh_in, float* dw, float* scratch, float* dummy, RangeGuard guard, const float* WfragN32,
                    const unsigned* wflag, unsigned wflag_ver) {
  MpWinNodeArgs a{};
  a.N = N; a.ntiles = cdiv(N, WTA);
  const int64_t per = win_tiles_per_wg(a.ntiles, ctx->num_cu, 8);
  a.tiles_per_wg = (int)per;
  a.dP = dP; a.dH = dh_out; a.h = h; a.csc_ptr = csc_ptr; a.rec = reinterpret_cast<const float4*>(rec);
  a.WfragN = WfragN; a.dh = dh_in; a.partial = scratch; a.dummy = dummy; a.guard = guard;
  const int grid = (int)cdiv(a.ntiles, per);
  const bool h2 = mp_win_bwd_h2();
#define NODE(HH, DW)                                                                                                    \
  switch (E) {                                                                                                          \
    case 1: hipLaunchKernelGGL((mp_win_bwd_node_kernel<1, HH, DW>), dim3(grid), dim3(WTHREADS), node_lds_bytes(E, HH), st, a); break; \
    case 2: hipLaunchKernelGGL((mp_win_bwd_node_kernel<2, HH, DW>), dim3(grid), dim3(WTHREADS), node_lds_bytes(E, HH), st, a); break; \
    case 3: hipLaunchKernelGGL((mp_win_bwd_node_kernel<3, HH, DW>), dim3(grid), dim3(WTHREADS), node_lds_bytes(E, HH), st, a); break; \
  }
  a.WfragN32 = WfragN32; a.wflag = wflag; a.wflag_ver = wflag_ver;
  {
    ProfScope ps(ctx, st, "mp_win_bwd_node");
    if (dw) {
      if (h2) { NODE(true, true) } else { NODE(false, true) }
    } else {
      if (h2) { NODE(true, false) } else { NODE(false, false) }
    }
    NG_HIP(ctx, hipGetLastError());
  }
#undef NODE
  if (!dw) return NG_OK;
  ProfScope ps(ctx, st, "reduce_partials");
  return reduce_or_defer(ctx, st, scratch, grid, (int64_t)E * WF * WF, dw, 2, WF, E, WF, (int64_t)E * WF * WF);
}

bool mp_win_bwd_supported(int F, int E, int K) {
  return F == WF && E >= 1 && E <= 3 && K % 4 == 0 && K >= 4 && K <= 16;
}

int mp_win_bwd_edge(ng_ctx* ctx, hipStream_t st, int64_t N, int K, int E, int act, const float* h,
                    const int32_t* nlist, const float* inv_degree, const float* WfragT, const float* s_save,
                    const float* dh_out, float* dP, float* de, int de_accum, float* dummy, RangeGuard guard,
                    const float* WfragT32, const unsigned* wflag, unsigned wflag_ver) {
  if (mp_win_bwd_h2() && guard.word && sw().mp_w16 && mp_win16_bwd_edge_supported(E, K))
    return mp_win16_bwd_edge_launch(ctx, st, N, K, E, act, h, nlist, inv_degree, WfragT, s_save, dh_out, dP, de, de_accum, dummy, guard,
                                    WfragT32, wflag, wflag_ver);
  MpWinEdgeArgs a{};
  a.N = N; a.K = K; a.ntiles = cdiv(N, WTA);
  const int64_t per = win_tiles_per_wg(a.ntiles, ctx->num_cu, 8);
  a.tiles_per_wg = (int)per;
  a.dH = dh_out; a.S = act == NG_ACT_NONE ? nullptr : s_save; a.rowscale = inv_degree; a.h = h;
  a.nlist = nlist; a.WfragT = WfragT; a.dP = dP; a.de = de; a.dummy = dummy; a.act = act;
  a.accumulate = de_accum; a.guard = guard;
  const int grid = (int)cdiv(a.ntiles, per);
  const size_t lds = edge_lds_bytes(K, E);
  const bool h2 = mp_win_bwd_h2();
#define EDGE(HH)                                                                                                  \
  switch (E) {                                                                                                    \
    case 1: hipLaunchKernelGGL((mp_win_bwd_edge_kernel<1, HH>), dim3(grid), dim3(WTHREADS), lds, st, a); break;   \
    case 2: hipLaunchKernelGGL((mp_win_bwd_edge_kernel<2, HH>), dim3(grid), dim3(WTHREADS), lds, st, a); break;   \
    case 3: hipLaunchKernelGGL((mp_win_bwd_edge_kernel<3, HH>), dim3(grid), dim3(WTHREADS), lds, st, a); break;   \
  }
  a.WfragT32 = WfragT32; a.wflag = wflag; a.wflag_ver = wflag_ver;
  {
    ProfScope ps(ctx, st, "mp_win_bwd_edge");
    if (h2) { EDGE(true) } else { EDGE(false) }
    NG_HIP(ctx, hipGetLastError());
  }
#undef EDGE
  return NG_OK;
}

bool mp_win_bwd_enabled(int F, int E, int K) { return mp_win_bwd_supported(F, E, K) && !sw().mp_layered; }

int mp_win_bwd(ng_ctx* ctx, hipStream_t st, int64_t N, int K, int E, int act, const float* h, const int32_t* nlist,
               const float* e, const float* inv_degree, const float* w, const float* s_save, const int32_t* csc_ptr,
               const int32_t* csc_edge, const float* dh_out, float* dh_in, float* de, int de_accum, float* dw,
               const float* csc_rec) {
  const int KF = E * WF;
  const size_t dw_scr = dw ? mp_win_node_scratch_floats(ctx, E) : 0;
  const bool h2 = mp_win_bwd_h2();
  const bool guarded = h2;
  RangeGuard guard{nullptr, 0};
  if (guarded) {
    guard = range_guard_begin(ctx);
    if (!guard.word) return NG_ERR_NOMEM;
  }
  const size_t img_floats = (size_t)4 * KF * WF + 16;
  bool have = false;
  float* imgs = (float*)cached_image(ctx, w, h2 ? 8 : 14, img_floats * 4, &have);
  const bool cached = imgs != nullptr;
  const size_t rec_floats = csc_rec ? 0 : (size_t)N * K * 4;
  float* ws = (float*)workspace(ctx, (size_t)((cached ? 0 : img_floats) + N * WF + rec_floats + dw_scr + 64) * 4);
  if (!ws) return NG_ERR_NOMEM;
  if (!cached) { imgs = ws; ws += img_floats; have = false; }
  float* WfragT = imgs;
  float* WfragN = WfragT + KF * WF;
  float* WfragT32 = WfragN + KF * WF;
  float* WfragN32 = WfragT32 + KF * WF;
  unsigned* wflag = cached && guarded ? reinterpret_cast<unsigned*>(WfragN32 + KF * WF) : nullptr;
  float* dP = ws;
  float* rec = dP + N * WF;
  float* scr = rec + rec_floats;
  float* dummy = scr + dw_scr;
  if (dw)
    if (float* dscr = deferred_partials(ctx, dw_scr)) scr = dscr;
  int rc = NG_OK;
  if (!have) {
    if (h2) {
      const PackJob j = mpw_bwd_job(E, w, WfragT, WfragN, guarded ? WfragT32 : nullptr, guarded ? WfragN32 : nullptr, wflag, guard);
      rc = pack_launch(ctx, st, j);
      if (rc == NG_OK && cached) cache_set_job(ctx, w, 8, j);
    } else {
      rc = mpw_pack2(ctx, st, E, w, 2, WfragT, 1, WfragN);
      if (cached) have = false;
    }
  }
  if (rc) return rc;
  const unsigned wver = pack_flag_version(ctx);
  rc = mp_win_bwd_edge(ctx, st, N, K, E, act, h, nlist, inv_degree, WfragT, s_save, dh_out, dP, de, de_accum, dummy, guard,
                       WfragT32, wflag, wver);
  if (rc) return rc;
  if (!csc_rec) {
    rc = mp_win_records(ctx, st, N, K, E, csc_ptr, csc_edge, e, rec);
    if (rc) return rc;
    csc_rec = rec;
  }
  return mp_win_bwd_node(ctx, st, N, E, h, dP, csc_ptr, csc_rec, WfragN, dh_out, dh_in, dw, scr, dummy, guard, WfragN32, wflag, wver);
}

}
```

nmrgnn_amd/csrc/ng_internal.h:

```cpp
#pragma once
#include <algorithm>

#include "ng_common.h"

namespace ng {

RangeGuard range_guard_begin(ng_ctx* ctx);
__device__ __forceinline__ void range_guard_raise(RangeGuard g, bool bad) {
  if (bad) __hip_atomic_store(g.word, g.epoch, __ATOMIC_RELAXED, __HIP_MEMORY_SCOPE_AGENT);
}
__device__ __forceinline__ bool range_guard_raised(RangeGuard g) {
  return __hip_atomic_load(g.word, __ATOMIC_RELAXED, __HIP_MEMORY_SCOPE_AGENT) == g.epoch;
}
__device__ __forceinline__ bool wimage_flag_raised(const unsigned* wflag) { return wflag && wflag[0] == wflag[1]; }
__device__ __forceinline__ bool not_finite(float v) { return !(fabsf(v) < INFINITY); }

struct LiveEdges {
  const int32_t* perm = nullptr;
  const int32_t* n_live = nullptr;
};

int dense_fwd(ng_ctx* ctx, hipStream_t st, int64_t M, int Kin, int Nout, int act, const float* X,
              const float* W, const float* b, const float* rowscale, const float* R, float* Y,
              float* S, const char* tag = "dense_fwd");
// ... 31 lines not shown
bool dense_grad_uses_h2(int64_t M, int Kin, int Nout);

bool edge_fused_supported(int H, int E, int Le);
int edge_fused_fwd(ng_ctx* ctx, hipStream_t st, int64_t n_edges, int E, const float* d_src,
                   const float* d_eff, const float* centers, float gap, const float* const* W,
                   const float* const* b, float* e_out, float* z_save, LiveEdges live = LiveEdges());
int edge_fused_fwd_f32(ng_ctx* ctx, hipStream_t st, int64_t n_edges, int E, const float* d_src,
                       const float* d_eff, const float* centers, float gap, const float* const* W,
                       const float* const* b, float* e_out, float* z_save, bool tape_blocked, const RangeGuard* guard,
                       LiveEdges live = LiveEdges());

int mp_plain_weights(ng_ctx* ctx, hipStream_t st, int64_t M, int F, int E, const float* w, float* scratch, int trans, const float** Wp);
int mp_repack_w(ng_ctx* ctx, hipStream_t st, int F, int E, const float* w, float* Wp);

int mp_generic_fwd(ng_ctx* ctx, hipStream_t st, int64_t N, int K, int F, int E, int act, int residual, const float* h,
                   const int32_t* row_ptr, const int32_t* col, const float* e, const float* inv_degree, const float* w,
                   float* h_out, float* A_save, float* s_save);
int mp_generic_bwd(ng_ctx* ctx, hipStream_t st, int64_t N, int K, int F, int E, int act, const float* h,
                   const int32_t* row_ptr, const int32_t* col, const int32_t* row_of, const float* e,
                   const float* inv_degree, const float* w, const float* A_save, const float* s_save,
                   const int32_t* csc_ptr, const int32_t* csc_edge, const float* dh_out, float* dh_in, float* de,
                   int de_accum, float* dw, const float* csc_rec = nullptr, int64_t nnz = 0);
int csr_aggregate(ng_ctx* ctx, hipStream_t st, int64_t N, int K, int F, int E, const float* h, const int32_t* row_ptr,
                  const int32_t* col, const float* e, float* A);

}

namespace ng {
struct TallArgs {
  int64_t N;
  const float* X;
  int ldx, k_valid;
  const float* S_in;
  const float* rs_in;
  int act_in;
  float* dP_out;
  const float* Wfrag;
  const float* bias;
  const float* rowscale;
  int act;
  float* S_save;
  const float* resid;
  float* out;
  int ldo, n_valid;
};
bool tall_gemm_supported(int kpad, int npad);
int tall_pack(ng_ctx* ctx, hipStream_t st, int k_in, int n_out, int kpad, int npad, int sk, int so,
              const float* w, float* out);
int tall_gemm(ng_ctx* ctx, hipStream_t st, int kpad, int npad, const TallArgs& a, bool prologue,
              const char* tag);

bool tall_tn_supported(int ka, int kb);
size_t tall_tn_scratch_floats(ng_ctx* ctx, int ka_valid);
int tall_tn(ng_ctx* ctx, hipStream_t st, int64_t N, const float* A, int lda, int ka_valid, const float* B,
            int ldb, int kb_valid, const float* S_in, int act_in, float* dW, float* db, int w_map, int F,
            int E, float* scratch, const char* tag);

bool knn_cells_supported(int G, int n, int K);
int knn_cells(ng_ctx* ctx, hipStream_t st, int G, int n, int K, float scale, const float* pos, int32_t* nlist, float* edges,
              float* inv_degree, const float* box = nullptr, int triclinic = 0);

bool mp_win_supported(int F, int E, int K);
bool mp_win_enabled(int F, int E, int K);
int mpw_pack(ng_ctx* ctx, hipStream_t st, int E, int mode, const float* w, float* out);
int mpw_pack2(ng_ctx* ctx, hipStream_t st, int E, const float* w, int mode_a, float* out_a, int mode_b, float* out_b);
inline int64_t win_tiles_per_wg(int64_t ntiles, int num_cu, int first_align) {
  const int64_t base = std::max<int64_t>(cdiv(ntiles, num_cu), 1);
  const int64_t want = std::min<int64_t>(num_cu, ntiles);
  for (int align = first_align; align > 1; align >>= 1) {
    const int64_t per = cdiv(base, align) * align;
    if (cdiv(ntiles, per) * 10 >= want * 9) return per;
  }
  return base;
}

bool agg_win_supported(int F, int E, int K);
int agg_win_rows();
int egrad_win(ng_ctx* ctx, hipStream_t st, int64_t N, int K, int F, int E, const float* h, const int32_t* nlist,
              const float* dA, float* de, int accumulate);
int agg_win(ng_ctx* ctx, hipStream_t st, int64_t N, int K, int F, int E, const float* h, const int32_t* nlist,
            const float* e, float* A);
PackJob mpw_bwd_job(int E, const float* w, float* outT, float* outN, float* f32T, float* f32N, unsigned* flag, RangeGuard guard);
bool mp_win16_bwd_edge_supported(int E, int K);
int mp_win16_bwd_edge_launch(ng_ctx* ctx, hipStream_t st, int64_t N, int K, int E, int act, const float* h, const int32_t* nlist,
                             const float* inv_degree, const float* WfragT, const float* s_save, const float* dh_out, float* dP,
                             float* de, int de_accum, float* dummy, RangeGuard guard, const float* WfragT32, const unsigned* wflag,
                             unsigned wflag_ver);
bool mp_win16_supported(int E, int K);
int mp_win16_launch(ng_ctx* ctx, hipStream_t st, int64_t N, int K, int E, int act, int residual, const float* h,
                    const int32_t* nlist, const float* e, const float* inv_degree, const float* Wfrag, const float* Wf32,
                    const unsigned* wflag, RangeGuard guard, float* h_out, float* s_save);
bool mp_wave_wanted(const ng_ctx* ctx, int64_t N, int E, int K);
int mp_wave_launch(ng_ctx* ctx, hipStream_t st, int64_t N, int K, int act, int residual, const float* h, const int32_t* nlist,
                   const float* e, const float* inv_degree, const float* Wfrag, const float* Wf32, const unsigned* wflag,
                   RangeGuard guard, float* h_out, float* s_save);
int mp_win_fwd(ng_ctx* ctx, hipStream_t st, int64_t N, int K, int E, int act, int residual, const float* h,
               const int32_t* nlist, const float* e, const float* inv_degree, const float* w, float* h_out,
               float* s_save);

bool mp_win_bwd_supported(int F, int E, int K);
int mp_win_bwd_edge(ng_ctx* ctx, hipStream_t st, int64_t N, int K, int E, int act, const float* h,
                    const int32_t* nlist, const float* inv_degree, const float* WfragT, const float* s_save,
                    const float* dh_out, float* dP, float* de, int de_accum, float* dummy, RangeGuard guard,
                    const float* WfragT32, const unsigned* wflag = nullptr, unsigned wflag_ver = 0);

int mp_win_records(ng_ctx* ctx, hipStream_t st, int64_t N, int K, int E, const int32_t* csc_ptr,
                   const int32_t* csc_edge, const float* e, float* rec, const int32_t* row_of = nullptr, int64_t n_entries = 0);
int mp_aggregate_padded(ng_ctx* ctx, hipStream_t st, int64_t N, int K, int F, int E, const float* h, const int32_t* nlist,
                        const float* e, float* A);
size_t mp_win_node_scratch_floats(ng_ctx* ctx, int E);
int mp_win_bwd_node(ng_ctx* ctx, hipStream_t st, int64_t N, int E, const float* h, const float* dP,
                    const int32_t* csc_ptr, const float* rec, const float* WfragN, const float* dh_out,
                    float* dh_in, float* dw, float* scratch, float* dummy, RangeGuard guard, const float* WfragN32,
                    const unsigned* wflag = nullptr, unsigned wflag_ver = 0);

bool mp_win_bwd_enabled(int F, int E, int K);
int mp_win_bwd(ng_ctx* ctx, hipStream_t st, int64_t N, int K, int E, int act, const float* h, const int32_t* nlist,
               const float* e, const float* inv_degree, const float* w, const float* s_save, const int32_t* csc_ptr,
               const int32_t* csc_edge, const float* dh_out, float* dh_in, float* de, int de_accum, float* dw,
               const float* csc_rec);

bool head_fast_supported(int Fh, int C);
int head_loss_graphs_per_wg(ng_ctx* ctx, int G, int Fh, int C, int64_t max_graph_atoms);
int head_loss_launch(ng_ctx* ctx, hipStream_t st, int64_t N, int G, int Fh, int C, int gpw, const float* g, uint64_t seed,
                     uint64_t offset, float keep, bool draw, float* mask_out, const float* Wout, const float* bout,
                     const float* atoms, const float* pstd, const float* pavg, const int32_t* gptr, const float* y,
                     const float* w, float gweight, float* peaks, float* dg, float* partial);
int head_loss_reduce(ng_ctx* ctx, hipStream_t st, const float* partial, int nb, int Fh, int C, float* dWout, float* dbout,
                     float* loss_out);
bool head_fwd_fast_supported(int Fh, int C);
int head_fwd_fast(ng_ctx* ctx, hipStream_t st, int64_t N, int Fh, int C, const float* g, const float* mask,
                  const float* Wout, const float* bout, const float* atoms, const float* pstd,
                  const float* pavg, float* peaks,
                  uint64_t seed = 0, uint64_t offset = 0, float keep = 1.f, float* mask_out = nullptr);
int head_bwd_fast(ng_ctx* ctx, hipStream_t st, int64_t N, int Fh, int C, const float* g, const float* mask,
                  const float* Wout, const float* atoms, const float* pstd, const float* dpeaks, float* dg,
                  float* dWout, float* dbout);
bool embed_bwd_fast_supported(int F, int C);
int embed_bwd_fast(ng_ctx* ctx, hipStream_t st, int64_t N, int C, int F, const float* atoms, const float* dh0,
                   float* dWemb);

}
```

nmrgnn_amd/csrc/node_ops.hip:

```cpp
#include <algorithm>
#include <type_traits>

#include "mfma_gemm.cuh"
#include "ng_internal.h"
#include "reduce.cuh"
#include "rng.cuh"

namespace ng {

constexpr int MAX_E = 8;
constexpr int MAX_C = 32;

struct LoadElem {
  const float* p;
  int ld;
  __device__ __forceinline__ float operator()(int64_t r, int c) const { return p[r * ld + c]; }
};
struct LoadHeadX {
  const float* g;
  const float* mask;
  int Fh;
  __device__ __forceinline__ float operator()(int64_t r, int f) const {
    if (f == Fh) return 1.0f;
    const float x = g[r * Fh + f];
// ... 522 lines not shown

__global__ __launch_bounds__(256) void loss_final_kernel(int G, const float* __restrict__ per_graph,
                                                         float* __restrict__ loss_out) {
  __shared__ float red[256];
  float s = 0.f;
  for (int i = threadIdx.x; i < G; i += 256) s += per_graph[i];
  red[threadIdx.x] = s;
  __syncthreads();
  for (int off = 128; off > 0; off >>= 1) {
    if (threadIdx.x < off) red[threadIdx.x] += red[threadIdx.x + off];
    __syncthreads();
  }
  if (threadIdx.x == 0) loss_out[0] = red[0] / (float)G;
}

__global__ void adam_kernel(int64_t n, float* __restrict__ p, const float* __restrict__ g,
                            float* __restrict__ m, float* __restrict__ v, float lr_t, float b1,
                            float b2, float eps, float gscale, const uint64_t* __restrict__ staged) {
  if (staged) lr_t = reinterpret_cast<const float*>(staged)[2];
  for (int64_t i = (int64_t)blockIdx.x * blockDim.x + threadIdx.x; i < n;
       i += (int64_t)gridDim.x * blockDim.x) {
    const float gi = g[i] * gscale;
    const float mi = b1 * m[i] + (1.0f - b1) * gi;
    const float vi = b2 * v[i] + (1.0f - b2) * gi * gi;
    m[i] = mi;
    v[i] = vi;
    p[i] -= lr_t * mi / (sqrtf(vi) + eps);
  }
}

__global__ void randn_kernel(uint64_t seed, uint64_t offset, float* __restrict__ out, int64_t n) {
  const int64_t n4 = (n + 3) / 4;
  for (int64_t q = (int64_t)blockIdx.x * blockDim.x + threadIdx.x; q < n4;
       q += (int64_t)gridDim.x * blockDim.x) {
    uint32_t r[4];
    philox4x32(seed, offset + (uint64_t)q, r);
    float z[4];
    const float r0 = sqrtf(-2.0f * logf(u01(r[0]))), t0 = 6.28318530717958648f * u01(r[1]);
    const float r1 = sqrtf(-2.0f * logf(u01(r[2]))), t1 = 6.28318530717958648f * u01(r[3]);
    z[0] = r0 * cosf(t0); z[1] = r0 * sinf(t0); z[2] = r1 * cosf(t1); z[3] = r1 * sinf(t1);
    for (int k = 0; k < 4; ++k)
      if (q * 4 + k < n) out[q * 4 + k] = z[k];
  }
}

__global__ void dropout_mask_kernel(uint64_t seed, uint64_t offset, float keep,
                                    float* __restrict__ out, int64_t n) {
  const int64_t n4 = (n + 3) / 4;
  const float inv = 1.0f / keep;
  for (int64_t q = (int64_t)blockIdx.x * blockDim.x + threadIdx.x; q < n4;
       q += (int64_t)gridDim.x * blockDim.x) {
    uint32_t r[4];
    philox4x32(seed, offset + (uint64_t)q, r);
    for (int k = 0; k < 4; ++k)
      if (q * 4 + k < n) out[q * 4 + k] = (u01(r[k]) <= keep) ? inv : 0.f;
  }
}

__global__ void add_scaled_kernel(int64_t n, const float* __restrict__ x,
                                  const float* __restrict__ y, float alpha,
                                  float* __restrict__ out) {
  for (int64_t i = (int64_t)blockIdx.x * blockDim.x + threadIdx.x; i < n;
       i += (int64_t)gridDim.x * blockDim.x)
    out[i] = x[i] + alpha * y[i];
}

__global__ void add_noise_kernel(uint64_t seed, uint64_t offset, int64_t n, const float* __restrict__ x, float alpha,
                                 float* __restrict__ out, const uint64_t* __restrict__ staged) {
  if (staged) seed = staged[0];
  const int64_t n4 = (n + 3) / 4;
  for (int64_t q = (int64_t)blockIdx.x * blockDim.x + threadIdx.x; q < n4;
       q += (int64_t)gridDim.x * blockDim.x) {
    uint32_t r[4];
    philox4x32(seed, offset + (uint64_t)q, r);
    float z[4];
    const float r0 = sqrtf(-2.0f * logf(u01(r[0]))), t0 = 6.28318530717958648f * u01(r[1]);
    const float r1 = sqrtf(-2.0f * logf(u01(r[2]))), t1 = 6.28318530717958648f * u01(r[3]);
    z[0] = r0 * cosf(t0); z[1] = r0 * sinf(t0); z[2] = r1 * cosf(t1); z[3] = r1 * sinf(t1);
    for (int k = 0; k < 4; ++k)
      if (q * 4 + k < n) out[q * 4 + k] = x[q * 4 + k] + alpha * z[k];
  }
}

__global__ void add_noise_live_kernel(uint64_t seed, uint64_t offset, int64_t n, const float* __restrict__ x,
                                      const float* __restrict__ y, float alpha, const int32_t* __restrict__ pos,
                                      float* __restrict__ out_c, const uint64_t* __restrict__ staged) {
  if (staged) seed = staged[0];
  const int64_t n4 = (n + 3) / 4;
  for (int64_t q = (int64_t)blockIdx.x * blockDim.x + threadIdx.x; q < n4;
       q += (int64_t)gridDim.x * blockDim.x) {
    float z[4];
    if (y) {
      for (int k = 0; k < 4; ++k) z[k] = q * 4 + k < n ? y[q * 4 + k] : 0.f;
    } else {
      uint32_t r[4];
      philox4x32(seed, offset + (uint64_t)q, r);
      const float r0 = sqrtf(-2.0f * logf(u01(r[0]))), t0 = 6.28318530717958648f * u01(r[1]);
      const float r1 = sqrtf(-2.0f * logf(u01(r[2]))), t1 = 6.28318530717958648f * u01(r[3]);
      z[0] = r0 * cosf(t0); z[1] = r0 * sinf(t0); z[2] = r1 * cosf(t1); z[3] = r1 * sinf(t1);
    }
    for (int k = 0; k < 4; ++k)
      if (q * 4 + k < n) {
        const int32_t p = pos[q * 4 + k];
        if (p >= 0) out_c[p] = x[q * 4 + k] + alpha * z[k];
      }
  }
}

static inline dim3 ew_grid(int64_t work_items) {
  return dim3((unsigned)std::max<int64_t>(1, std::min<int64_t>(cdiv(work_items, 256), 256 * 8)));
}

}

using namespace ng;

extern "C" int ng_randn(ng_ctx* ctx, void* stream, uint64_t seed, uint64_t offset, float* out,
                        int64_t n) {
  if (!ctx) return NG_ERR_INVALID;
  if (n == 0) return NG_OK;
  hipLaunchKernelGGL(randn_kernel, ew_grid((n + 3) / 4), dim3(256), 0, (hipStream_t)stream, seed,
                     offset, out, n);
  NG_HIP(ctx, hipGetLastError());
  return NG_OK;
}

extern "C" int ng_dropout_mask(ng_ctx* ctx, void* stream, uint64_t seed, uint64_t offset, float keep,
                               float* out, int64_t n) {
  if (!ctx) return NG_ERR_INVALID;
  NG_REQUIRE(ctx, keep > 0.f && keep <= 1.f, "dropout keep probability in (0,1]");
  if (n == 0) return NG_OK;
  hipLaunchKernelGGL(dropout_mask_kernel, ew_grid((n + 3) / 4), dim3(256), 0, (hipStream_t)stream,
                     seed, offset, keep, out, n);
  NG_HIP(ctx, hipGetLastError());
  return NG_OK;
}

extern "C" int ng_add_noise(ng_ctx* ctx, void* stream, uint64_t seed, uint64_t offset, int64_t n, const float* x,
                            float alpha, float* out) {
  if (!ctx) return NG_ERR_INVALID;
  if (n == 0) return NG_OK;
  hipLaunchKernelGGL(add_noise_kernel, ew_grid((n + 3) / 4), dim3(256), 0, (hipStream_t)stream, seed, offset, n, x,
                     alpha, out, ng::replay_state(ctx));
  NG_HIP(ctx, hipGetLastError());
  return NG_OK;
}

extern "C" int ng_add_noise_live(ng_ctx* ctx, void* stream, uint64_t seed, uint64_t offset, int64_t n, const float* x,
                                 const float* y, float alpha, const int32_t* pos, float* out_c) {
  if (!ctx) return NG_ERR_INVALID;
  if (n == 0) return NG_OK;
  NG_REQUIRE(ctx, x && pos && out_c, "add_noise_live: arguments");
  hipLaunchKernelGGL(add_noise_live_kernel, ew_grid((n + 3) / 4), dim3(256), 0, (hipStream_t)stream, seed, offset, n, x, y,
                     alpha, pos, out_c, ng::replay_state(ctx));
  NG_HIP(ctx, hipGetLastError());
  return NG_OK;
}

extern "C" int ng_add_scaled(ng_ctx* ctx, void* stream, int64_t n, const float* x, const float* y,
                             float alpha, float* out) {
  if (!ctx) return NG_ERR_INVALID;
  if (n == 0) return NG_OK;
  hipLaunchKernelGGL(add_scaled_kernel, ew_grid(n), dim3(256), 0, (hipStream_t)stream, n, x, y,
                     alpha, out);
  NG_HIP(ctx, hipGetLastError());
  return NG_OK;
}

extern "C" int ng_embed_fwd(ng_ctx* ctx, void* stream, int64_t N, int C, int F, const float* atoms,
                            const float* Wemb, float* h0) {
  if (!ctx) return NG_ERR_INVALID;
  NG_REQUIRE(ctx, F % 4 == 0, "embed: F % 4");
  if (N == 0) return NG_OK;
  ProfScope ps(ctx, (hipStream_t)stream, "embed_fwd");
  const dim3 grid = ew_grid(N * (F / 4));
  if (C <= 16 && F == 64 && !sw().head_generic)
    hipLaunchKernelGGL((embed_fwd_rows_kernel<16>), grid, dim3(256), 0, (hipStream_t)stream, N, C, atoms, Wemb, h0);
  else if (C <= 16 && F == 128 && !sw().head_generic)
    hipLaunchKernelGGL((embed_fwd_rows_kernel<32>), grid, dim3(256), 0, (hipStream_t)stream, N, C, atoms, Wemb, h0);
  else if (C <= 16 && F == 256 && !sw().head_generic)
    hipLaunchKernelGGL((embed_fwd_rows_kernel<64>), grid, dim3(256), 0, (hipStream_t)stream, N, C, atoms, Wemb, h0);
  else
    hipLaunchKernelGGL(embed_fwd_kernel, grid, dim3(256), 0, (hipStream_t)stream, N, C, F, atoms, Wemb, h0);
  NG_HIP(ctx, hipGetLastError());
  return NG_OK;
}

extern "C" int ng_embed_bwd(ng_ctx* ctx, void* stream, int64_t N, int C, int F, const float* atoms,
// ... 16 lines not shown
  LoadElem fy{dh0, F};
  const dim3 grid((unsigned)nb, (unsigned)cdiv(items, 256 * SMALL_TN_ITEMS));
  hipLaunchKernelGGL((small_tn_kernel<LoadElem, LoadElem>), grid, dim3(256),
                     (size_t)64 * (C + F) * 4, st, N, C, F, rows, fx, fy, partial);
  launch_reduce_z(st, partial, (int)nb, items, dWemb);
  NG_HIP(ctx, hipGetLastError());
  return NG_OK;
}

extern "C" int ng_mp_aggregate(ng_ctx* ctx, void* stream, int64_t N, int K, int F, int E,
                               const float* h, const int32_t* nlist, const float* e, float* A) {
  if (!ctx) return NG_ERR_INVALID;
  return aggregate(ctx, (hipStream_t)stream, N, K, F, E, h, nlist, e, A);
}

extern "C" int ng_mp_layer_fwd(ng_ctx* ctx, void* stream, int64_t N, int K, int F, int E, int act,
                               int residual, const float* h, const int32_t* nlist, const float* e,
                               const float* inv_degree, const float* w, float* h_out, float* A_save,
                               float* s_save) {
  if (!ctx) return NG_ERR_INVALID;
  hipStream_t st = (hipStream_t)stream;
  NG_REQUIRE(ctx, (E * F) % 8 == 0, "mp_layer: (E*F) % 8");
  if (N > 0 && mp_win_enabled(F, E, K)) {
    if (A_save) {
      const int rc = aggregate(ctx, st, N, K, F, E, h, nlist, e, A_save);
      if (rc) return rc;
    }
    return mp_win_fwd(ctx, st, N, K, E, act, residual, h, nlist, e, inv_degree, w, h_out, s_save);
  }
  if (E > MAX_E)
    return mp_generic_fwd(ctx, st, N, K, F, E, act, residual, h, nullptr, nlist, e, inv_degree, w, h_out, A_save, s_save);
  if (mp_gg_supported(N, F, E, K) || mp_gw_infer_ok(ctx, N, K, F, E, false, A_save != nullptr))
    return mp_gg_fwd(ctx, st, N, K, F, E, act, residual, h, nullptr, nlist, e, inv_degree, w, h_out, s_save, A_save);
  const int64_t KF = (int64_t)E * F;
  const size_t need = (size_t)(KF * F + (A_save ? 0 : N * KF)) * 4;
  float* ws = (float*)workspace(ctx, need);
  if (!ws) return NG_ERR_NOMEM;
  const float* Wp = nullptr;
  float* A = A_save ? A_save : ws + KF * F;
  int rc = mp_plain_weights(ctx, st, N, F, E, w, ws, 0, &Wp);
  if (rc) return rc;
  rc = aggregate(ctx, st, N, K, F, E, h, nlist, e, A);
  if (rc) return rc;
  return dense_fwd(ctx, st, N, (int)KF, F, act, A, Wp, nullptr, inv_degree, residual ? h : nullptr,
                   h_out, s_save,
                   "mp_update_fwd");
}

extern "C" int ng_mp_layer_wants_aggregate(int F, int E, int K) {
  if (mp_win_bwd_enabled(F, E, K)) return 0;
  return 1;
}

extern "C" int ng_mp_edge_records(ng_ctx* ctx, void* stream, int64_t N, int K, int E, const int32_t* csc_ptr,
                                  const int32_t* csc_edge, const float* e, float* rec) {
  if (!ctx) return NG_ERR_INVALID;
  NG_REQUIRE(ctx, E >= 1 && E <= 3, "edge records hold at most 3 edge features");
  return mp_win_records(ctx, (hipStream_t)stream, N, K, E, csc_ptr, csc_edge, e, rec);
}

extern "C" int ng_mp_layer_bwd_rec(ng_ctx* ctx, void* stream, int64_t N, int K, int F, int E, int act,
                                   const float* h, const int32_t* nlist, const float* e,
                                   const float* inv_degree, const float* w, const float* A_save,
                                   const float* s_save, const int32_t* csc_ptr, const int32_t* csc_edge,
                                   const float* dh_out, float* dh_in, float* de, int de_accum,
                                   float* dw, const float* csc_rec);

extern "C" int ng_mp_layer_bwd(ng_ctx* ctx, void* stream, int64_t N, int K, int F, int E, int act,
                               const float* h, const int32_t* nlist, const float* e,
                               const float* inv_degree, const float* w, const float* A_save,
                               const float* s_save, const int32_t* csc_ptr, const int32_t* csc_edge,
                               const float* dh_out, float* dh_in, float* de, int de_accum,
                               float* dw) {
  return ng_mp_layer_bwd_rec(ctx, stream, N, K, F, E, act, h, nlist, e, inv_degree, w, A_save, s_save, csc_ptr,
                             csc_edge, dh_out, dh_in, de, de_accum, dw, nullptr);
}

extern "C" int ng_mp_layer_bwd_rec(ng_ctx* ctx, void* stream, int64_t N, int K, int F, int E, int act,
                                   const float* h, const int32_t* nlist, const float* e,
                                   const float* inv_degree, const float* w, const float* A_save,
                                   const float* s_save, const int32_t* csc_ptr, const int32_t* csc_edge,
                                   const float* dh_out, float* dh_in, float* de, int de_accum,
                                   float* dw, const float* csc_rec) {
  if (!ctx) return NG_ERR_INVALID;
  hipStream_t st = (hipStream_t)stream;
  NG_REQUIRE(ctx, act == NG_ACT_NONE || s_save, "mp_layer_bwd: s_save required for an activation");
  NG_REQUIRE(ctx, F % 4 == 0 && F >= 16 && F <= 256 && (256 % (F / 4)) == 0,
             "mp_layer_bwd: F in {16,32,64,128,256}");
  NG_REQUIRE(ctx, E >= 1 && E <= 64, "mp_layer_bwd: edge_feature_size <= 64");
  if (N > 0 && mp_win_bwd_enabled(F, E, K))
    return mp_win_bwd(ctx, st, N, K, E, act, h, nlist, e, inv_degree, w, s_save, csc_ptr, csc_edge, dh_out, dh_in, de,
                      de_accum, dw, csc_rec);
  return mp_generic_bwd(ctx, st, N, K, F, E, act, h, nullptr, nlist, nullptr, e, inv_degree, w, A_save, s_save, csc_ptr,
                        csc_edge, dh_out, dh_in, de, de_accum, dw, E <= 3 ? csc_rec : nullptr);
}

extern "C" int ng_head_fwd(ng_ctx* ctx, void* stream, int64_t N, int Fh, int C, const float* g,
                           const float* drop_mask, const float* Wout, const float* bout,
                           const float* atoms, const float* peak_std, const float* peak_avg,
                           float* peaks) {
  if (!ctx) return NG_ERR_INVALID;
  NG_REQUIRE(ctx, C >= 1 && C <= MAX_C, "head: number of elements <= 32");
  if (N == 0) return NG_OK;
  if (head_fwd_fast_supported(Fh, C))
    return head_fwd_fast(ctx, (hipStream_t)stream, N, Fh, C, g, drop_mask, Wout, bout, atoms, peak_std,
                         peak_avg, peaks);
  ProfScope ps(ctx, (hipStream_t)stream, "head_fwd");
  hipLaunchKernelGGL(head_fwd_kernel, dim3((unsigned)cdiv(N, 256)), dim3(256), (size_t)Fh * C * 4,
                     (hipStream_t)stream, N, Fh, C, g, drop_mask, Wout, bout, atoms, peak_std,
                     peak_avg, peaks);
  NG_HIP(ctx, hipGetLastError());
  return NG_OK;
}

extern "C" int ng_head_fwd_dropout(ng_ctx* ctx, void* stream, int64_t N, int Fh, int C, const float* g, uint64_t seed,
                                   uint64_t offset, float keep, float* mask_out, const float* Wout, const float* bout,
                                   const float* atoms, const float* peak_std, const float* peak_avg, float* peaks) {
  if (!ctx) return NG_ERR_INVALID;
  NG_REQUIRE(ctx, C >= 1 && C <= MAX_C, "head: number of elements <= 32");
  NG_REQUIRE(ctx, keep > 0.f && keep <= 1.f, "dropout keep probability in (0,1]");
  NG_REQUIRE(ctx, mask_out, "head_fwd_dropout: mask_out [N,Fh] required (the backward reads it)");
  if (N == 0) return NG_OK;
  if (head_fwd_fast_supported(Fh, C) && Fh % 4 == 0)
    return head_fwd_fast(ctx, (hipStream_t)stream, N, Fh, C, g, nullptr, Wout, bout, atoms, peak_std, peak_avg, peaks,
                         seed, offset, keep, mask_out);
  NG_REQUIRE(ctx, !ctx->replay_armed, "head_fwd_dropout: this head shape cannot be replayed (seed is a launch argument)");
  const int rc = ng_dropout_mask(ctx, stream, seed, offset, keep, mask_out, N * Fh);
  if (rc) return rc;
  return ng_head_fwd(ctx, stream, N, Fh, C, g, mask_out, Wout, bout, atoms, peak_std, peak_avg, peaks);
}

extern "C" int ng_head_loss_blocks(ng_ctx* ctx, int G, int Fh, int C, int64_t max_graph_atoms) {
  if (!ctx) return 0;
  const int gpw = head_loss_graphs_per_wg(ctx, G, Fh, C, max_graph_atoms);
  return gpw ? (int)cdiv(G, gpw) : 0;
}

extern "C" int ng_head_loss_bwd(ng_ctx* ctx, void* stream, int64_t N, int G, int Fh, int C, int64_t max_graph_atoms,
                                const float* g, uint64_t seed, uint64_t offset, float keep, float* mask_out,
                                const float* Wout, const float* bout, const float* atoms, const float* peak_std,
                                const float* peak_avg, const int32_t* graph_ptr, const float* y, const float* w,
                                float grad_weight, float* peaks, float* dg, float* partial) {
  if (!ctx) return NG_ERR_INVALID;
  NG_REQUIRE(ctx, C >= 1 && C <= MAX_C, "head: number of elements <= 32");
  NG_REQUIRE(ctx, keep > 0.f && keep <= 1.f, "dropout keep probability in (0,1]");
  NG_REQUIRE(ctx, N >= 1 && G >= 1, "head_loss_bwd: at least one graph and one atom");
  NG_REQUIRE(ctx, g && Wout && bout && atoms && peak_std && peak_avg && graph_ptr && y && w && peaks && dg && partial,
             "head_loss_bwd: arguments");
  const int gpw = head_loss_graphs_per_wg(ctx, G, Fh, C, max_graph_atoms);
  if (!gpw) { ctx->err = "head_loss_bwd: shape not supported (ng_head_loss_blocks == 0)"; return NG_ERR_UNSUPPORTED; }
  return head_loss_launch(ctx, (hipStream_t)stream, N, G, Fh, C, gpw, g, seed, offset, keep, keep < 1.f, mask_out, Wout, bout,
                          atoms, peak_std, peak_avg, graph_ptr, y, w, grad_weight, peaks, dg, partial);
}

extern "C" int ng_head_loss_reduce(ng_ctx* ctx, void* stream, const float* partial, int nb, int Fh, int C, float* dWout,
                                   float* dbout, float* loss_out) {
  if (!ctx) return NG_ERR_INVALID;
  NG_REQUIRE(ctx, partial && nb >= 1 && dWout && dbout && loss_out && C >= 1 && C <= MAX_C, "head_loss_reduce: arguments");
  return head_loss_reduce(ctx, (hipStream_t)stream, partial, nb, Fh, C, dWout, dbout, loss_out);
}

extern "C" int ng_head_bwd(ng_ctx* ctx, void* stream, int64_t N, int Fh, int C, const float* g,
                           const float* drop_mask, const float* Wout, const float* atoms,
                           const float* peak_std, const float* dpeaks, float* dg, float* dWout,
                           float* dbout) {
  if (!ctx) return NG_ERR_INVALID;
  hipStream_t st = (hipStream_t)stream;
  NG_REQUIRE(ctx, C >= 1 && C <= MAX_C, "head: number of elements <= 32");
  NG_REQUIRE(ctx, (dWout == nullptr) == (dbout == nullptr), "head_bwd: dWout and dbout are both given or both NULL");
  const int64_t items = (int64_t)Fh * C + C;
  if (N == 0) {
    if (!dWout) return NG_OK;
    NG_HIP(ctx, hipMemsetAsync(dWout, 0, (size_t)Fh * C * 4, st));
    NG_HIP(ctx, hipMemsetAsync(dbout, 0, (size_t)C * 4, st));
    return NG_OK;
// ... 139 lines not shown
```

nmrgnn_amd/engine.py:

```python
from __future__ import annotations

import ctypes as C
import os

import numpy as np
import torch

from . import _lib
from ._lib import ptr, ptr_array
from .graph import GraphBatch
from .params import ParamStore

ACT = {None: 0, "linear": 0, "softplus": 1, "relu": 2, "tanh": 3}
DROPOUT_RATE = 0.2
FUSED_TAIL_MAX_ATOMS = 16384


def rbf_grid(low, high, count):
    lo, hi = np.float32(low), np.float32(high)
    delta = (hi - lo) / np.float32(count - 1)
    c = (lo + delta * np.arange(count, dtype=np.float32)).astype(np.float32)
    c[-1] = hi
    return c, float(np.float32(c[1] - c[0]))

# ... 209 lines not shown
            self._ck(lib.ng_fc_head_fwd(h, st, N, F, self.Lf, self.C, self.fc_act, ptr(hs[-1]), ptr_array(Wfc), ptr_array(Bfc),
                                        ptr(P["out/kernel"]), ptr(P["out/bias"]), ptr(batch.atoms), ptr(self.peak_std),
                                        ptr(self.peak_avg), ptr(peaks)), "ng_fc_head_fwd")
            return peaks
        fx = [hs[-1]]
        for t in range(self.Lf - 1):
            fx.append(self._new(N, F))
        Fh = F // 2
        g = self._new(N, Fh)
        self._ck(lib.ng_fc_block_fwd(h, st, N, F, self.Lf, self.fc_act, ptr(fx[0]), ptr_array(Wfc),
                                     ptr_array(Bfc), ptr_array(fx[1:]), ptr(g)), "ng_fc_block_fwd")
        mask = None
        peaks = self._new(N)
        loss_t = dpeaks = dg = head_partial = None
        nb = 0
        if loss is not None and self.fuse_head_loss and dropout_mask is None:
            nb = int(lib.ng_head_loss_blocks(h, batch.G, Fh, self.C, batch.max_graph_atoms))
        if nb > 0:
            y, w, gw = loss
            keep = (1.0 - DROPOUT_RATE) if (training and self.use_dropout) else 1.0
            loss_t, dg = self._new(1), self._new(N, Fh)
            head_partial = self._new(nb, Fh * self.C + self.C + 1)
            self._ck(lib.ng_head_loss_bwd(h, st, N, batch.G, Fh, self.C, batch.max_graph_atoms, ptr(g), seed, 1 << 40, keep,
                                          None, ptr(P["out/kernel"]), ptr(P["out/bias"]), ptr(batch.atoms),
                                          ptr(self.peak_std), ptr(self.peak_avg), ptr(batch.graph_ptr), ptr(y), ptr(w),
                                          float(gw), ptr(peaks), ptr(dg), ptr(head_partial)),
                     "ng_head_loss_bwd")
        elif training and self.use_dropout and dropout_mask is None:
            mask = self._new(N, Fh)
            self._ck(lib.ng_head_fwd_dropout(h, st, N, Fh, self.C, ptr(g), seed, 1 << 40, 1.0 - DROPOUT_RATE, ptr(mask),
                                             ptr(P["out/kernel"]), ptr(P["out/bias"]), ptr(batch.atoms),
                                             ptr(self.peak_std), ptr(self.peak_avg), ptr(peaks)), "ng_head_fwd_dropout")
        else:
            if training and self.use_dropout:
                mask = dropout_mask.reshape(N, Fh).contiguous()
            self._ck(lib.ng_head_fwd(h, st, N, Fh, self.C, ptr(g), ptr(mask), ptr(P["out/kernel"]),
                                     ptr(P["out/bias"]), ptr(batch.atoms), ptr(self.peak_std),
                                     ptr(self.peak_avg), ptr(peaks)), "ng_head_fwd")
        if loss is not None and nb == 0:
            y, w, gw = loss
            loss_t, dpeaks = self.loss_l2(batch, y, w, peaks)
            if gw != 1.0:
                dpeaks.mul_(gw)
        if tape:
            tp = Tape()
            tp.loss, tp.dpeaks, tp.dg, tp.head_partial = loss_t, dpeaks, dg, head_partial
            tp.batch, tp.d_eff, tp.z_save, tp.e = batch, d_eff, z_save, e
            tp.z_layout = z_layout
            tp.edge_path, tp.live, tp.table = path, live, table
            tp.inputs_only = inputs_only
            tp.h, tp.A, tp.S, tp.fx, tp.g, tp.drop_mask, tp.peaks = hs, As, Ss, fx, g, mask, peaks
            self.tape = tp
        return peaks

    EDGE_TABLE_POINTS = 4096

    def _table_points(self):
        return self.EDGE_TABLE_POINTS if self.E <= 4 else self.EDGE_TABLE_POINTS // 2

    def _edge_weights(self):
        P = self.params
        return [P[f"edge_fc/{t}/kernel"] for t in range(self.Le)], [P[f"edge_fc/{t}/bias"] for t in range(self.Le)]

    def _edge_grads(self, view=None):
        view = view or self.params.g
        return [view(f"edge_fc/{t}/kernel") for t in range(self.Le)], [view(f"edge_fc/{t}/bias") for t in range(self.Le)]

    def _edge_mlp_fwd(self, n, d_src, d_eff, e, tape, perm=None, rows=None):
        lib, h, st = self.lib, self.ctx.handle, self._st()
        z, z_layout = None, 0
        if tape:
            z = self._new(self.Le - 1, n, self.H)
            z_layout = int(lib.ng_edge_tape_layout(self.H, self.E, self.Le, self.fc_act, n))
        W, B = self._edge_weights()
        if perm is None:
            self._ck(lib.ng_edge_mlp_fwd(h, st, n, self.H, self.E, self.Le, self.fc_act, ptr(d_src), ptr(d_eff), ptr(self.centers),
                                         self.gap, ptr_array(W), ptr_array(B), ptr(e), ptr(z)), "ng_edge_mlp_fwd")
        else:
            self._ck(lib.ng_edge_mlp_fwd_live(h, st, n, self.H, self.E, self.Le, self.fc_act, ptr(d_src), ptr(d_eff), ptr(perm),
                                              ptr(rows), ptr(self.centers), self.gap, ptr_array(W), ptr_array(B), ptr(e), ptr(z)),
                     "ng_edge_mlp_fwd_live")
        return z, z_layout

    def _edge_mlp_bwd(self, n, d_src, d_eff, z, z_layout, de, grads, perm=None, rows=None):
        lib, h, st = self.lib, self.ctx.handle, self._st()
        W, _ = self._edge_weights()
        dW, dB = grads
        if perm is None:
            self._ck(lib.ng_edge_mlp_bwd_tape(h, st, n, self.H, self.E, self.Le, self.fc_act, ptr(d_src), ptr(d_eff),
                                              ptr(self.centers), self.gap, ptr_array(W), ptr(z), ptr(de), ptr_array(dW),
                                              ptr_array(dB), z_layout), "ng_edge_mlp_bwd")
        else:
            self._ck(lib.ng_edge_mlp_bwd_live(h, st, n, self.H, self.E, self.Le, self.fc_act, ptr(d_src), ptr(d_eff), ptr(perm),
                                              ptr(rows), ptr(self.centers), self.gap, ptr_array(W), ptr(z), ptr(de),
                                              ptr_array(dW), ptr_array(dB), z_layout), "ng_edge_mlp_bwd_live")

    def _edge_table_build(self, batch, live, d_eff, tape, training):
        lib, h, st = self.lib, self.ctx.handle, self._st()
        pos, n_live = (None, None) if live is None else (live[1], live[3])
        ne, E, T = batch.n_edges, self.E, self._table_points()
        d_src = batch.edges.reshape(-1)
        tol = -1.0 if self.edge_table_force_fallback else float(self.edge_table_tol)
        reuse = live is not None and self._frozen and not tape and not training and not self.edge_table_force_fallback
        gate = torch.empty(8, dtype=torch.int32, device=self.device)
        kept = reuse and self._table_cache is not None and self._table_cache["key"] == (self._wgen, T, E)
        rng = self._new(4)
        self._ck(lib.ng_edge_table_range(h, st, ne, E, ptr(d_src), ptr(d_eff), ptr(pos), None, 0.25 if reuse and not kept else 0.0,
                                         ptr(rng)), "ng_edge_table_range")
        if kept:
            c = self._table_cache
            self._ck(lib.ng_edge_table_check(h, st, T, E, None, 0.0, ptr(c["rng"]), ptr(rng), ptr(n_live), 2 * T,
                                             ptr(c["gate"]), ptr(gate)), "ng_edge_table_check")
            return {"e_all": c["e_all"], "rng": c["rng"], "gate": gate, "T": T, "kept": c, "cover": rng}
        d_tab, ones = self._new(2 * T), self._new(2 * T)
        perm_tab = None if live is None else torch.empty(2 * T, dtype=torch.int32, device=self.device)
        self._ck(lib.ng_edge_table_points(h, st, T, 1, ptr(rng), ptr(d_tab), ptr(ones), ptr(perm_tab)), "ng_edge_table_points")
        e_all = self._new(2 * T, E)
        z_tab, z_layout = self._edge_mlp_fwd(2 * T, ones, d_tab, e_all, tape, perm_tab, self._rows_2t)
        self._ck(lib.ng_edge_table_check(h, st, T, E, ptr(e_all), tol, ptr(rng), None, ptr(n_live), 2 * T, None, ptr(gate)),
                 "ng_edge_table_check")
        if live is None and int(gate[0].item()) != 0:
            return None
        kept = None
        if reuse:
            kept = self._table_cache = {"key": (self._wgen, T, E), "e_all": e_all, "rng": rng, "gate": gate}
        return {"e_all": e_all, "rng": rng, "gate": gate, "T": T, "d_tab": d_tab, "ones": ones, "perm_tab": perm_tab,
                "z_tab": z_tab, "z_layout": z_layout, "kept": kept, "cover": rng}

    def _edge_table_backward(self, tp, de, grads):
        tb, b = tp.table, tp.batch
        T = tb["T"]
        pos = None if tp.live is None else tp.live[1]
        de_tab = self._new(2 * T, self.E)
        self._ck(self.lib.ng_edge_table_scatter(self.ctx.handle, self._st(), b.n_edges, self.E, T, 2 * T, ptr(b.edges), ptr(tp.d_eff),
                                                ptr(pos), ptr(tb["rng"]), ptr(de), ptr(de_tab)), "ng_edge_table_scatter")
        self._edge_mlp_bwd(2 * T, tb["ones"], tb["d_tab"], tb["z_tab"], tb["z_layout"], de_tab, grads, tb["perm_tab"], tb["gate"][2:])

    def edge_table_report(self, table=None):
        tb = table if table is not None else (self.tape.table if self.tape is not None else None)
        if tb is None:
            raise RuntimeError("edge_table_report: no edge-function table (no taped call, or the call went per edge)")
        g = tb["gate"].cpu().numpy()
        return bool(g[0]), float(g[4:6].view(np.float32)[0]), float(g[4:6].view(np.float32)[1])

    def backward(self, dpeaks, on_node_grads=None, edge_grad=None, param_grad=True):
        if not param_grad:
            if edge_grad is None:
                raise ValueError("backward(param_grad=False) needs edge_grad: without parameter gradients it is the only output")
            if on_node_grads is not None:
                raise ValueError("backward(param_grad=False): on_node_grads hands on parameter gradients, and none are formed")
            if dpeaks is None:
                raise ValueError("backward(param_grad=False) needs dpeaks: the fused head + loss launch already formed the "
                                 "head's weight-gradient partials")
        if edge_grad is not None:
            b = self.tape.batch if self.tape is not None else None
            if b is not None and (edge_grad.dtype != torch.float32 or edge_grad.device != self.device
                                  or not edge_grad.is_contiguous() or tuple(edge_grad.shape) != tuple(b.edges.shape)):
                raise ValueError("backward: edge_grad must be a contiguous float32 tensor on the engine's device, "
                                 "shaped like batch.edges")
        tp = self.tape
        if tp is None:
            raise RuntimeError("backward() without forward(training=True)")
        if tp.inputs_only and param_grad:
            raise RuntimeError("backward(param_grad=True) on a tape of forward(keep_tape=\"inputs\"): the edge MLP kept no "
                               "activations; call backward(param_grad=False, edge_grad=...)")
        lib, h, st = self.lib, self.ctx.handle, self._st()
        self._ck(lib.ng_defer_reductions(h, st, 1 if self.defer_reductions and param_grad else 0), "ng_defer_reductions")
        if self.cache_images:
            self._ck(lib.ng_weights_frozen(h, self._id), "ng_weights_frozen")
        try:
            self._backward(tp, dpeaks, on_node_grads, lib, h, st, edge_grad, bool(param_grad))
        finally:
            if self.cache_images:
                lib.ng_weights_frozen(h, 0)
            self._ck(lib.ng_defer_reductions(h, st, 0), "ng_defer_reductions")

    def _backward(self, tp, dpeaks, on_node_grads, lib, h, st, edge_grad=None, param_grad=True):
        P = self.params
        wg = P.g if param_grad else (lambda name: None)
        warr = ptr_array if param_grad else (lambda ts: None)
        b = tp.batch
        N, K, F, E = b.N, b.K, self.F, self.E
        Fh = F // 2
        ne = b.n_edges
        self._ck(lib.ng_ctx_set_graph_span(h, b.max_graph_atoms), "ng_ctx_set_graph_span")
        if dpeaks is None and tp.dg is not None:
            dg = tp.dg
            self._ck(lib.ng_head_loss_reduce(h, st, ptr(tp.head_partial), tp.head_partial.shape[0], Fh, self.C,
                                             ptr(P.g("out/kernel")), ptr(P.g("out/bias")), ptr(tp.loss)),
                     "ng_head_loss_reduce")
        else:
            if tp.dg is not None:
                raise RuntimeError("backward(dpeaks) after forward(loss=...): the head's backward already ran with the "
                                   "loss gradient; call backward(None)")
            if dpeaks is None:
                dpeaks = tp.dpeaks
            if dpeaks is None:
                raise RuntimeError("backward(None) without forward(loss=...)")
            dpeaks = dpeaks.contiguous()
            dg = self._new(N, Fh)
            self._ck(lib.ng_head_bwd(h, st, N, Fh, self.C, ptr(tp.g), ptr(tp.drop_mask),
                                     ptr(P["out/kernel"]), ptr(b.atoms), ptr(self.peak_std),
                                     ptr(dpeaks), ptr(dg), ptr(wg("out/kernel")), ptr(wg("out/bias"))),
                     "ng_head_bwd")
        dx = self._new(N, F)
        Wfc = [P[f"fc/{t}/kernel"] for t in range(self.Lf)]
        ns = int(lib.ng_fc_block_scratch_floats(N, F, self.Lf))
        scratch = self._new(ns) if ns else None
        self._ck(lib.ng_fc_block_bwd(h, st, N, F, self.Lf, self.fc_act, ptr_array(tp.fx), ptr(tp.g),
                                     ptr_array(Wfc), ptr(dg), ptr(dx),
                                     warr([wg(f"fc/{t}/kernel") for t in range(self.Lf)]),
                                     warr([wg(f"fc/{t}/bias") for t in range(self.Lf)]),
                                     ptr(scratch)), "ng_fc_block_bwd")
        csc_ptr, csc_edge = b.csc()
        de = self._new(ne, E)
        rec = None
        if E <= 3 and not b.is_csr:
            rec = self._new(ne, 4)
            self._ck(lib.ng_mp_edge_records(h, st, N, K, E, ptr(csc_ptr), ptr(csc_edge), ptr(tp.e), ptr(rec)),
                     "ng_mp_edge_records")
        dh = dx
        for l in reversed(range(self.L)):
            dhn = self._new(N, F)
            if b.is_csr:
                self._ck(lib.ng_mp_layer_bwd_csr(h, st, N, ne, F, E, self.mp_act, ptr(tp.h[l]), ptr(b.row_ptr),
                                                 ptr(b.nlist), ptr(b.row_of), ptr(tp.e), ptr(b.inv_degree),
                                                 ptr(P[f"mp/{l}/w"]), ptr(tp.A[l]), ptr(tp.S[l]), ptr(csc_ptr),
                                                 ptr(csc_edge), ptr(dh), ptr(dhn), ptr(de),
                                                 0 if l == self.L - 1 else 1, ptr(wg(f"mp/{l}/w"))),
                         "ng_mp_layer_bwd_csr")
                dh = dhn
                continue
            self._ck(lib.ng_mp_layer_bwd_rec(h, st, N, K, F, E, self.mp_act, ptr(tp.h[l]), ptr(b.nlist_c),
                                         ptr(tp.e), ptr(b.inv_degree), ptr(P[f"mp/{l}/w"]),
                                         ptr(tp.A[l]), ptr(tp.S[l]), ptr(csc_ptr), ptr(csc_edge),
                                         ptr(dh), ptr(dhn), ptr(de), 0 if l == self.L - 1 else 1,
                                         ptr(wg(f"mp/{l}/w")), ptr(rec)), "ng_mp_layer_bwd")
            dh = dhn
        if not param_grad:
            self._edge_dinput(tp, de, edge_grad)
            self.tape = None
            return
        self._ck(lib.ng_embed_bwd(h, st, N, self.C, F, ptr(b.atoms), ptr(dh),
                                  ptr(P.g("embed/kernel"))), "ng_embed_bwd")
        self._ck(lib.ng_flush_reductions(h, st), "ng_flush_reductions")
        if on_node_grads is not None:
            on_node_grads()
        if tp.edge_path == "slots":
            self._edge_mlp_bwd(ne, b.edges, tp.d_eff, tp.z_save, tp.z_layout, de, self._edge_grads())
        elif tp.edge_path == "live":
            perm, _, d_c, n_live = tp.live
            self._edge_mlp_bwd(ne, d_c, tp.d_eff, tp.z_save, tp.z_layout, de, self._edge_grads(), perm, n_live)
        elif tp.edge_path == "table_host":
            self._edge_table_backward(tp, de, self._edge_grads())
        else:
            names = [f"edge_fc/{t}/{k}" for t in range(self.Le) for k in ("kernel", "bias")]
            o0 = min(P.offsets[n] for n in names)
            o1 = max(P.offsets[n] + int(np.prod(P.shapes[n])) for n in names)
            tmp = self._new(o1 - o0)
            tv = lambda n: tmp[P.offsets[n] - o0:P.offsets[n] - o0 + int(np.prod(P.shapes[n]))]
            perm, _, d_c, _ = tp.live
            self._edge_mlp_bwd(ne, d_c, tp.d_eff, tp.z_save, tp.z_layout, de, self._edge_grads(tv), perm, tp.table["gate"][1:])
            self._edge_table_backward(tp, de, self._edge_grads())
            blk = P.grad[o0:o1]
            self._ck(lib.ng_add_scaled(h, st, o1 - o0, ptr(blk), ptr(tmp), 1.0, ptr(blk)), "ng_add_scaled")
        if edge_grad is not None:
            self._edge_dinput(tp, de, edge_grad)
        self.tape = None

    def _edge_dinput(self, tp, de, out):
        b = tp.batch
        if tp.live is not None:
            perm, _, d_src, n_live = tp.live
        else:
            perm = n_live = None
            d_src = b.edges.reshape(-1)
        if not (self.edge_grad_table and tp.table is not None and tp.edge_path in ("table", "table_host")):
            self._jgate = None
            self._edge_mlp_dinput(b.n_edges, d_src, tp.d_eff, perm, n_live, de, None, out)
            return
        J_all, rng, jgate = self._edge_jacobian_table(tp)
        self._jgate = jgate
        lib, h, st = self.lib, self.ctx.handle, self._st()
        if tp.edge_path == "table":
            self._edge_mlp_dinput(b.n_edges, d_src, tp.d_eff, perm, jgate[1:], de, None, out)
        elif int(jgate[0].item()) != 0:
            self._edge_mlp_dinput(b.n_edges, d_src, tp.d_eff, None, None, de, None, out)
            return
        self._ck(lib.ng_edge_table_dinput(h, st, b.n_edges, self.E, tp.table["T"], ptr(b.edges), ptr(tp.d_eff),
                                          ptr(None if tp.live is None else tp.live[1]), ptr(rng), ptr(J_all), ptr(jgate), ptr(de),
                                          ptr(out)), "ng_edge_table_dinput")

    def _edge_mlp_dinput(self, n, d_src, d_eff, perm, n_live, de, J_out, out):
        W, B = self._edge_weights()
        self._ck(self.lib.ng_edge_mlp_dinput(self.ctx.handle, self._st(), n, self.H, self.E, self.Le, self.fc_act,
                                             ptr(d_src), ptr(d_eff), ptr(perm), ptr(n_live), ptr(self.centers), self.gap,
                                             ptr_array(W), ptr_array(B), ptr(de), ptr(J_out), ptr(out)), "ng_edge_mlp_dinput")

    def _edge_jacobian_table(self, tp):
        lib, h, st = self.lib, self.ctx.handle, self._st()
        tb, E, T = tp.table, self.E, tp.table["T"]
        n_live = None if tp.live is None else tp.live[3]
        c = None if self.edge_table_force_fallback else tb["kept"]
        jgate = torch.empty(8, dtype=torch.int32, device=self.device)
        if c is None or "J_all" not in c:
            tol = -1.0 if self.edge_table_force_fallback else float(self.edge_grad_table_tol)
            if "d_tab" in tb:
                d_tab, ones, perm_tab = tb["d_tab"], tb["ones"], tb["perm_tab"]
            else:
                d_tab, ones = self._new(2 * T), self._new(2 * T)
                perm_tab = None if tp.live is None else torch.empty(2 * T, dtype=torch.int32, device=self.device)
                self._ck(lib.ng_edge_table_points(h, st, T, 1, ptr(tb["rng"]), ptr(d_tab), ptr(ones), ptr(perm_tab)),
                         "ng_edge_table_points")
            J_all, de0, dd0 = self._new(2 * T, E), torch.zeros(2 * T, E, dtype=torch.float32, device=self.device), self._new(2 * T)
            self._edge_mlp_dinput(2 * T, ones, d_tab, perm_tab, None if perm_tab is None else self._rows_2t, de0, J_all, dd0)
            own = jgate if c is None else torch.empty(8, dtype=torch.int32, device=self.device)
            self._ck(lib.ng_edge_table_check(h, st, T, E, ptr(J_all), tol, ptr(tb["rng"]), None, ptr(n_live), 2 * T,
                                             ptr(tb["gate"] if c is None else c["gate"]), ptr(own)), "ng_edge_table_check")
            if c is None:
                return J_all, tb["rng"], jgate
            c["J_all"], c["jgate"] = J_all, own
        self._ck(lib.ng_edge_table_check(h, st, T, E, None, 0.0, ptr(c["rng"]), ptr(tb["cover"]), ptr(n_live), 2 * T,
                                         ptr(c["jgate"]), ptr(jgate)), "ng_edge_table_check")
        return c["J_all"], c["rng"], jgate

    def edge_grad_table_report(self):
        if self._jgate is None:
            raise RuntimeError("edge_grad_table_report: the last backward took no Jacobian table (edge_grad_table off, no "
                               "edge_grad, or a per-edge tape)")
        g = self._jgate.cpu().numpy()
        return bool(g[0]), float(g[4:6].view(np.float32)[0]), float(g[4:6].view(np.float32)[1])

    def loss_l2(self, batch, y, w, peaks):
        loss = self._new(1)
        dpred = self._new(batch.N)
# ... 31 lines not shown
```

Baseline: 43.70 million.

## Fuse de abs-max reduction into message-passing backward and vectorize reductions

The last message-passing backward layer now computes per-workgroup abs-max of the edge gradient while writing it, and the edge MLP backward consumes these block maxima instead of running a separate max pass over de. The edge-backward partial-sum reduce kernel is also vectorized to float4 with four outputs per lane and deeper unrolling. The noise-add kernel is restructured to coalesce loads via an LDS transpose. These remove a separate reduction launch and pass over de, at the cost of extra template instantiations and a fixed-size maxima buffer.

```diff
diff --git a/include/nmrgnn_hip.h b/include/nmrgnn_hip.h
--- a/include/nmrgnn_hip.h
+++ b/include/nmrgnn_hip.h
@@ -84,6 +84,12 @@
                          const float* d_src_c, const float* d_eff_c, const int32_t* perm, const int32_t* n_live,
                          const float* centers, float gap, const float* const* W, const float* z_save,
                          const float* de, float* const* dW, float* const* db, int tape_layout);
+enum { NG_DE_ABSMAX_LEN = 1024 };
+int ng_de_absmax_len(void);
+int ng_edge_mlp_bwd_live_max(ng_ctx*, void* stream, int64_t n_slots, int H, int E, int Le, int act,
+                             const float* d_src_c, const float* d_eff_c, const int32_t* perm, const int32_t* n_live,
+                             const float* centers, float gap, const float* const* W, const float* z_save,
+                             const float* de, float* const* dW, float* const* db, int tape_layout, const float* de_absmax);
 
 int ng_edge_mlp_dinput(ng_ctx*, void* stream, int64_t n_slots, int H, int E, int Le, int act, const float* d_src,
                        const float* d_eff, const int32_t* perm, const int32_t* n_live, const float* centers, float gap,
@@ -147,6 +153,12 @@
                     const float* w, const float* A_save, const float* s_save,
                     const int32_t* csc_ptr, const int32_t* csc_edge, const float* dh_out,
                     float* dh_in, float* de, int de_accum, float* dw, const float* csc_rec);
+int ng_mp_layer_bwd_de_max_ok(ng_ctx*, int64_t N, int K, int F, int E);
+int ng_mp_layer_bwd_rec_max(ng_ctx*, void* stream, int64_t N, int K, int F, int E, int act,
+                    const float* h, const int32_t* nlist, const float* e, const float* inv_degree,
+                    const float* w, const float* A_save, const float* s_save,
+                    const int32_t* csc_ptr, const int32_t* csc_edge, const float* dh_out,
+                    float* dh_in, float* de, int de_accum, float* dw, const float* csc_rec, float* de_absmax);
 
 int ng_mp_aggregate_csr(ng_ctx*, void* stream, int64_t N, int F, int E, const float* h,
                         const int32_t* row_ptr, const int32_t* col, const float* e, float* A);
diff --git a/nmrgnn_amd/_lib.py b/nmrgnn_amd/_lib.py
--- a/nmrgnn_amd/_lib.py
+++ b/nmrgnn_amd/_lib.py
@@ -65,6 +65,9 @@
                                     C.POINTER(_vp), C.POINTER(_vp), _vp, _vp]),
     "ng_edge_mlp_bwd_live": (_int, [_vp, _vp, _i64, _int, _int, _int, _int, _vp, _vp, _vp, _vp, _vp, _f,
                                     C.POINTER(_vp), _vp, _vp, C.POINTER(_vp), C.POINTER(_vp), _int]),
+    "ng_de_absmax_len": (_int, []),
+    "ng_edge_mlp_bwd_live_max": (_int, [_vp, _vp, _i64, _int, _int, _int, _int, _vp, _vp, _vp, _vp, _vp, _f,
+                                        C.POINTER(_vp), _vp, _vp, C.POINTER(_vp), C.POINTER(_vp), _int, _vp]),
     "ng_edge_mlp_dinput": (_int, [_vp, _vp, _i64, _int, _int, _int, _int, _vp, _vp, _vp, _vp, _vp, _f,
                                   C.POINTER(_vp), C.POINTER(_vp), _vp, _vp, _vp]),
     "ng_positions_grad": (_int, [_vp, _vp, _i64, _int, _vp, _vp, _vp, _vp, _f, _vp, _vp, _vp]),
@@ -89,6 +92,9 @@
                                _vp, _vp, _vp, _vp, _vp, _vp, _vp, _int, _vp]),
     "ng_mp_layer_bwd_rec": (_int, [_vp, _vp, _i64, _int, _int, _int, _int, _vp, _vp, _vp, _vp, _vp,
                                _vp, _vp, _vp, _vp, _vp, _vp, _vp, _int, _vp, _vp]),
+    "ng_mp_layer_bwd_de_max_ok": (_int, [_vp, _i64, _int, _int, _int]),
+    "ng_mp_layer_bwd_rec_max": (_int, [_vp, _vp, _i64, _int, _int, _int, _int, _vp, _vp, _vp, _vp, _vp,
+                               _vp, _vp, _vp, _vp, _vp, _vp, _vp, _int, _vp, _vp, _vp]),
     "ng_mp_edge_records": (_int, [_vp, _vp, _i64, _int, _int, _vp, _vp, _vp, _vp]),
     "ng_mp_aggregate_csr": (_int, [_vp, _vp, _i64, _int, _int, _vp, _vp, _vp, _vp, _vp]),
     "ng_mp_layer_fwd_csr": (_int, [_vp, _vp, _i64, _i64, _int, _int, _int, _int, _vp, _vp, _vp, _vp, _vp, _vp,
diff --git a/nmrgnn_amd/csrc/edge_bwd_h2.hip b/nmrgnn_amd/csrc/edge_bwd_h2.hip
--- a/nmrgnn_amd/csrc/edge_bwd_h2.hip
+++ b/nmrgnn_amd/csrc/edge_bwd_h2.hip
@@ -342,7 +342,7 @@
 int edge_bwd_h2_launch(ng_ctx* ctx, hipStream_t st, int64_t n_edges, int E, const float* d_src, const float* d_eff,
                        const float* centers, float gap, const float* const* W, const float* z_save, const float* de,
                        char* wt_img, float* partial, int part_stride, int grid, int tape_blocked, RangeGuard guard,
-                       LiveEdges live) {
+                       LiveEdges live, const float* de_absmax) {
   float* blockmax = reinterpret_cast<float*>(wt_img + HX_WT_BYTES + 16);
   int nb_max = 0;
   bool have_wt = false;
@@ -357,7 +357,10 @@
       if (int rc = pack_launch(ctx, st, j)) return rc;
       if (cached_wt) cache_set_job(ctx, W[1], 13, j);
     }
-    if (n_edges * E <= HX_DIRECT_MAX && (reinterpret_cast<uintptr_t>(de) & 15) == 0) {
+    if (de_absmax) {
+      nb_max = DE_ABSMAX_LEN;
+      blockmax = const_cast<float*>(de_absmax);
+    } else if (n_edges * E <= HX_DIRECT_MAX && (reinterpret_cast<uintptr_t>(de) & 15) == 0) {
       nb_max = -(int)(n_edges * E);
       blockmax = const_cast<float*>(de);
     } else {
diff --git a/nmrgnn_amd/csrc/edge_fused.h b/nmrgnn_amd/csrc/edge_fused.h
--- a/nmrgnn_amd/csrc/edge_fused.h
+++ b/nmrgnn_amd/csrc/edge_fused.h
@@ -17,7 +17,7 @@
 int edge_fused_bwd(ng_ctx* ctx, hipStream_t st, int64_t n_edges, int E, const float* d_src,
                    const float* d_eff, const float* centers, float gap, const float* const* W,
                    const float* z_save, const float* de, float* const* dW, float* const* db, int tape_layout = -1,
-                   LiveEdges live = LiveEdges());
+                   LiveEdges live = LiveEdges(), const float* de_absmax = nullptr);
 }
 
 #define NG_LDS_BARRIER()                                   \
@@ -39,5 +39,5 @@
 int edge_bwd_h2_launch(ng_ctx* ctx, hipStream_t st, int64_t n_edges, int E, const float* d_src, const float* d_eff,
                        const float* centers, float gap, const float* const* W, const float* z_save, const float* de,
                        char* wt_img, float* partial, int part_stride, int grid, int tape_blocked, RangeGuard guard,
-                       LiveEdges live = LiveEdges());
+                       LiveEdges live = LiveEdges(), const float* de_absmax = nullptr);
 }
diff --git a/nmrgnn_amd/csrc/edge_fused_bwd.hip b/nmrgnn_amd/csrc/edge_fused_bwd.hip
--- a/nmrgnn_amd/csrc/edge_fused_bwd.hip
+++ b/nmrgnn_amd/csrc/edge_fused_bwd.hip
@@ -315,44 +315,72 @@
 
 __global__ __launch_bounds__(1024) void edge_bwd_reduce_kernel(const float* __restrict__ partial, int n_wg,
                                                                int stride, int E, BwdOut o, const int32_t* __restrict__ n_live) {
-  __shared__ float red[16][64];
+  constexpr int V = 4;
+  __shared__ __attribute__((aligned(16))) float red[16][64 * V];
   const int total = bwd_part_floats(E);
   const int lane = threadIdx.x & 63, wv = threadIdx.x >> 6;
-  const int idx = blockIdx.x * 64 + lane;
-  float s = 0.f;
+  const int idx = (blockIdx.x * 64 + lane) * V;
+  float s[V];
+#pragma unroll
+  for (int e = 0; e < V; ++e) s[e] = 0.f;
   if (n_live && *n_live < 0) n_wg = 0;
+  auto load = [&](const float* q, float (&v)[V]) {
+    const float4 t = *reinterpret_cast<const float4*>(q);
+    v[0] = t.x; v[1] = t.y; v[2] = t.z; v[3] = t.w;
+  };
   if (idx < total) {
     const float* p = partial + idx;
     int w = wv;
+    for (; w + 240 < n_wg; w += 256) {
+      float v[16][V];
+#pragma unroll
+      for (int u = 0; u < 16; ++u) load(p + (int64_t)(w + 16 * u) * stride, v[u]);
+#pragma unroll
+      for (int u = 0; u < 16; ++u)
+#pragma unroll
+        for (int e = 0; e < V; ++e) s[e] += v[u][e];
+    }
     for (; w + 112 < n_wg; w += 128) {
-      float v[8];
-#pragma unroll
-      for (int u = 0; u < 8; ++u) v[u] = p[(int64_t)(w + 16 * u) * stride];
-#pragma unroll
-      for (int u = 0; u < 8; ++u) s += v[u];
-    }
-    for (; w < n_wg; w += 16) s += p[(int64_t)w * stride];
-  }
-  red[wv][lane] = s;
+      float v[8][V];
+#pragma unroll
+      for (int u = 0; u < 8; ++u) load(p + (int64_t)(w + 16 * u) * stride, v[u]);
+#pragma unroll
+      for (int u = 0; u < 8; ++u)
+#pragma unroll
+        for (int e = 0; e < V; ++e) s[e] += v[u][e];
+    }
+    for (; w < n_wg; w += 16) {
+      float v[V];
+      load(p + (int64_t)w * stride, v);
+#pragma unroll
+      for (int e = 0; e < V; ++e) s[e] += v[e];
+    }
+  }
+#pragma unroll
+  for (int e = 0; e < V; ++e) red[wv][lane * V + e] = s[e];
   __syncthreads();
   if (wv != 0 || idx >= total) return;
-  s = red[0][lane];
-#pragma unroll
-  for (int j = 1; j < 16; ++j) s += red[j][lane];
-  int r = idx;
-  if (r < 3 * FH * FH) { o.dW[r / (FH * FH)][r % (FH * FH)] = s; return; }
-  r -= 3 * FH * FH;
-  if (r < 3 * FH) { o.db[r / FH][r % FH] = s; return; }
-  r -= 3 * FH;
-  if (r < FH * E) { o.dWo[r] = s; return; }
-  r -= FH * E;
-  o.dbo[r] = s;
+#pragma unroll
+  for (int e = 0; e < V; ++e) {
+    float t = red[0][lane * V + e];
+#pragma unroll
+    for (int j = 1; j < 16; ++j) t += red[j][lane * V + e];
+    int r = idx + e;
+    if (r >= total) break;
+    if (r < 3 * FH * FH) { o.dW[r / (FH * FH)][r % (FH * FH)] = t; continue; }
+    r -= 3 * FH * FH;
+    if (r < 3 * FH) { o.db[r / FH][r % FH] = t; continue; }
+    r -= 3 * FH;
+    if (r < FH * E) { o.dWo[r] = t; continue; }
+    r -= FH * E;
+    o.dbo[r] = t;
+  }
 }
 
 int edge_fused_bwd(ng_ctx* ctx, hipStream_t st, int64_t n_edges, int E, const float* d_src,
                    const float* d_eff, const float* centers, float gap, const float* const* W,
                    const float* z_save, const float* de, float* const* dW, float* const* db, int tape_layout,
-                   LiveEdges live) {
+                   LiveEdges live, const float* de_absmax) {
   const int64_t ntiles = cdiv(n_edges, FTM);
   const int grid = (int)std::min<int64_t>(ntiles, (int64_t)ctx->num_cu);
   const int stride = (bwd_part_floats(E) + 3) / 4 * 4;
@@ -386,7 +414,7 @@
     const RangeGuard guard = range_guard_begin(ctx);
     if (!guard.word) return NG_ERR_NOMEM;
     int rc3 = edge_bwd_h2_launch(ctx, st, n_edges, E, d_src, d_eff, centers, gap, W, z_save, de,
-                     (char*)(partial + (size_t)nseg * grid * stride), partial, stride, grid, blocked ? 1 : 0, guard, live);
+                     (char*)(partial + (size_t)nseg * grid * stride), partial, stride, grid, blocked ? 1 : 0, guard, live, de_absmax);
     if (rc3) return rc3;
     n_part = nseg * grid;
     a.tape_blocked = blocked ? 1 : 0; a.zero_rows = n_part; a.guard = guard;
@@ -406,7 +434,7 @@
     BwdOut o;
     for (int l = 0; l < 3; ++l) { o.dW[l] = dW[l]; o.db[l] = db[l]; }
     o.dWo = dW[3]; o.dbo = db[3];
-    hipLaunchKernelGGL(edge_bwd_reduce_kernel, dim3((unsigned)cdiv(bwd_part_floats(E), 64)), dim3(1024), 0, st,
+    hipLaunchKernelGGL(edge_bwd_reduce_kernel, dim3((unsigned)cdiv(bwd_part_floats(E), 256)), dim3(1024), 0, st,
                        partial, n_part, stride, E, o, live.n_live);
     NG_HIP(ctx, hipGetLastError());
   }
diff --git a/nmrgnn_amd/csrc/edge_ops.hip b/nmrgnn_amd/csrc/edge_ops.hip
--- a/nmrgnn_amd/csrc/edge_ops.hip
+++ b/nmrgnn_amd/csrc/edge_ops.hip
@@ -369,13 +369,24 @@
                                     const float* d_src_c, const float* d_eff_c, const int32_t* perm, const int32_t* n_live,
                                     const float* centers, float gap, const float* const* W, const float* z_save,
                                     const float* de, float* const* dW, float* const* db, int tape_layout) {
+  return ng_edge_mlp_bwd_live_max(ctx, stream, n_slots, H, E, Le, act, d_src_c, d_eff_c, perm, n_live, centers, gap, W, z_save, de,
+                                  dW, db, tape_layout, nullptr);
+}
+
+extern "C" int ng_de_absmax_len(void) { return NG_DE_ABSMAX_LEN; }
+
+extern "C" int ng_edge_mlp_bwd_live_max(ng_ctx* ctx, void* stream, int64_t n_slots, int H, int E, int Le, int act,
+                                        const float* d_src_c, const float* d_eff_c, const int32_t* perm, const int32_t* n_live,
+                                        const float* centers, float gap, const float* const* W, const float* z_save,
+                                        const float* de, float* const* dW, float* const* db, int tape_layout,
+                                        const float* de_absmax) {
   if (!ctx) return NG_ERR_INVALID;
   if (int rc = check_edge_shape(ctx, H, E, Le, act)) return rc;
   NG_REQUIRE(ctx, z_save, "edge_mlp_bwd: saved activations required");
   NG_REQUIRE(ctx, n_slots > 0, "edge_mlp_bwd live view: n_slots > 0");
   if (int rc = check_live(ctx, n_slots, H, E, Le, act, perm, n_live)) return rc;
   return edge_fused_bwd(ctx, (hipStream_t)stream, n_slots, E, d_src_c, d_eff_c, centers, gap, W, z_save, de, dW, db,
-                        tape_layout, LiveEdges{perm, n_live});
+                        tape_layout, LiveEdges{perm, n_live}, de_absmax);
 }
 
 extern "C" int ng_edge_tape_layout(int H, int E, int Le, int act, int64_t n_edges) {
diff --git a/nmrgnn_amd/csrc/mp_win16_bwd.hip b/nmrgnn_amd/csrc/mp_win16_bwd.hip
--- a/nmrgnn_amd/csrc/mp_win16_bwd.hip
+++ b/nmrgnn_amd/csrc/mp_win16_bwd.hip
@@ -30,6 +30,7 @@
   const float* WfragT32;
   float* dP;
   float* de;
+  float* de_max;
   float* dummy;
   int act;
   int accumulate;
@@ -38,7 +39,7 @@
   unsigned wflag_ver;
 };
 
-template <int E, bool H2, int ACT = -1>
+template <int E, bool H2, int ACT = -1, bool BM = false>
 __device__ __forceinline__ void body(const Args& a) {
   const int act_ = ACT >= 0 ? ACT : a.act;
   constexpr int KF = E * WF;
@@ -56,7 +57,13 @@
   const int K = a.K;
   const int64_t T0 = (int64_t)blockIdx.x * a.tiles_per_wg;
   const int64_t T1 = std::min<int64_t>(T0 + a.tiles_per_wg, a.ntiles);
-  if (T0 >= T1) return;
+  if (BM)
+    for (int i = (int)gridDim.x + (int)blockIdx.x * WTHREADS + tid; i < DE_ABSMAX_LEN; i += (int)gridDim.x * WTHREADS) a.de_max[i] = 0.f;
+  if (T0 >= T1) {
+    if (BM && tid == 0) a.de_max[blockIdx.x] = 0.f;
+    return;
+  }
+  float mde = 0.f;
 
   const float4* src4 = reinterpret_cast<const float4*>(a.h);
   float4* win4 = reinterpret_cast<float4*>(win);
@@ -192,7 +199,11 @@
       const bool live = row < a.N && pc < K;
       float* dst = live ? a.de + (row * K + pc) * E : a.dummy;
 #pragma unroll
-      for (int n = 0; n < E; ++n) dst[n] = out[n] + p_de[n];
+      for (int n = 0; n < E; ++n) {
+        const float v = out[n] + p_de[n];
+        dst[n] = v;
+        if (BM && live) mde = fmaxf(mde, fabsf(v));
+      }
     }
     if (t + 1 < T1) commit(t + 1);
     idx_cur = p_idx;
@@ -200,13 +211,24 @@
     issue_de(t + 1 < T1 ? t + 1 : t);
     NG_LDS_BARRIER();
   }
-}
-
-template <int E>
+  if (BM) {
+#pragma unroll
+    for (int o = 32; o > 0; o >>= 1) mde = fmaxf(mde, __shfl_xor(mde, o, 64));
+    if (lane == 0) s_inv[wave] = mde;
+    __syncthreads();
+    if (tid == 0) {
+      float m = s_inv[0];
+      for (int w = 1; w < NW; ++w) m = fmaxf(m, s_inv[w]);
+      a.de_max[blockIdx.x] = m;
+    }
+  }
+}
+
+template <int E, bool BM>
 __global__ __launch_bounds__(WTHREADS) void mp_win16_bwd_edge_kernel(Args a) {
-  if (a.guard.word && (range_guard_raised(a.guard) || wimage_flag_raised(a.wflag))) body<E, false>(a);
-  else if (a.act == NG_ACT_SOFTPLUS) body<E, true, NG_ACT_SOFTPLUS>(a);
-  else body<E, true>(a);
+  if (a.guard.word && (range_guard_raised(a.guard) || wimage_flag_raised(a.wflag))) body<E, false, -1, BM>(a);
+  else if (a.act == NG_ACT_SOFTPLUS) body<E, true, NG_ACT_SOFTPLUS, BM>(a);
+  else body<E, true, -1, BM>(a);
 }
 
 }
@@ -216,27 +238,42 @@
 }
 
 bool mp_win16_bwd_edge_supported(int E, int K) { return E >= 1 && E <= 3 && K >= 1 && K <= 16; }
+
+static int mp_win16_bwd_edge_grid(const ng_ctx* ctx, int64_t N, int64_t* per_out) {
+  const int64_t ntiles = cdiv(N, (int64_t)w16b::WTA);
+  const int64_t per = win_tiles_per_wg(ntiles, ctx->num_cu, 4);
+  if (per_out) *per_out = per;
+  return (int)cdiv(ntiles, per);
+}
+
+bool mp_win16_bwd_edge_de_max_ok(const ng_ctx* ctx, int64_t N) {
+  return N > 0 && mp_win16_bwd_edge_grid(ctx, N, nullptr) <= DE_ABSMAX_LEN;
+}
 
 int mp_win16_bwd_edge_launch(ng_ctx* ctx, hipStream_t st, int64_t N, int K, int E, int act, const float* h, const int32_t* nlist,
                              const float* inv_degree, const float* WfragT, const float* s_save, const float* dh_out, float* dP,
                              float* de, int de_accum, float* dummy, RangeGuard guard, const float* WfragT32, const unsigned* wflag,
-                             unsigned wflag_ver) {
+                             unsigned wflag_ver, float* de_max) {
   using namespace w16b;
   Args a{};
   a.N = N; a.K = K; a.ntiles = cdiv(N, WTA);
-  const int64_t per = win_tiles_per_wg(a.ntiles, ctx->num_cu, 4);
+  int64_t per = 1;
+  const int grid = mp_win16_bwd_edge_grid(ctx, N, &per);
+  if (de_max && grid > DE_ABSMAX_LEN) return fail(ctx, NG_ERR_INVALID, "mp_win16_bwd_edge: more workgroups than de_max holds");
+  a.de_max = de_max;
   a.tiles_per_wg = (int)per;
   a.dH = dh_out; a.S = act == NG_ACT_NONE ? nullptr : s_save; a.rowscale = inv_degree; a.h = h;
   a.nlist = nlist; a.WfragT = WfragT; a.WfragT32 = WfragT32; a.dP = dP; a.de = de; a.dummy = dummy; a.act = act;
   a.accumulate = de_accum; a.guard = guard; a.wflag = wflag; a.wflag_ver = wflag_ver;
-  const int grid = (int)cdiv(a.ntiles, per);
   const size_t lds = mp_win16_bwd_edge_lds(E);
   ProfScope ps(ctx, st, "mp_win_bwd_edge");
-  switch (E) {
-    case 1: hipLaunchKernelGGL((mp_win16_bwd_edge_kernel<1>), dim3(grid), dim3(WTHREADS), lds, st, a); break;
-    case 2: hipLaunchKernelGGL((mp_win16_bwd_edge_kernel<2>), dim3(grid), dim3(WTHREADS), lds, st, a); break;
-    case 3: hipLaunchKernelGGL((mp_win16_bwd_edge_kernel<3>), dim3(grid), dim3(WTHREADS), lds, st, a); break;
-  }
+#define NG_W16B(EE)                                                                                              \
+  case EE:                                                                                                       \
+    if (de_max) hipLaunchKernelGGL((mp_win16_bwd_edge_kernel<EE, true>), dim3(grid), dim3(WTHREADS), lds, st, a); \
+    else hipLaunchKernelGGL((mp_win16_bwd_edge_kernel<EE, false>), dim3(grid), dim3(WTHREADS), lds, st, a);      \
+    break;
+  switch (E) { NG_W16B(1) NG_W16B(2) NG_W16B(3) }
+#undef NG_W16B
   NG_HIP(ctx, hipGetLastError());
   return NG_OK;
 }
diff --git a/nmrgnn_amd/csrc/mp_win_bwd.hip b/nmrgnn_amd/csrc/mp_win_bwd.hip
--- a/nmrgnn_amd/csrc/mp_win_bwd.hip
+++ b/nmrgnn_amd/csrc/mp_win_bwd.hip
@@ -714,7 +714,7 @@
                                   float4* __restrict__ rec, const int32_t* __restrict__ row_of) {
   const int64_t nnz = csc_ptr[N];
   const int64_t stride = (int64_t)gridDim.x * blockDim.x;
-  for (int64_t p0 = (int64_t)blockIdx.x * blockDim.x + threadIdx.x; p0 < nnz; p0 += 4 * stride) {
+  for (int64_t p0 = (int64_t)xcd_tile(blockIdx.x, gridDim.x) * blockDim.x + threadIdx.x; p0 < nnz; p0 += 4 * stride) {
     int eid[4];
 #pragma unroll
     for (int u = 0; u < 4; ++u) eid[u] = csc_edge[std::min<int64_t>(p0 + u * stride, nnz - 1)];
@@ -805,10 +805,11 @@
 int mp_win_bwd_edge(ng_ctx* ctx, hipStream_t st, int64_t N, int K, int E, int act, const float* h,
                     const int32_t* nlist, const float* inv_degree, const float* WfragT, const float* s_save,
                     const float* dh_out, float* dP, float* de, int de_accum, float* dummy, RangeGuard guard,
-                    const float* WfragT32, const unsigned* wflag, unsigned wflag_ver) {
+                    const float* WfragT32, const unsigned* wflag, unsigned wflag_ver, float* de_max) {
   if (mp_win_bwd_h2() && guard.word && sw().mp_w16 && mp_win16_bwd_edge_supported(E, K))
     return mp_win16_bwd_edge_launch(ctx, st, N, K, E, act, h, nlist, inv_degree, WfragT, s_save, dh_out, dP, de, de_accum, dummy, guard,
-                                    WfragT32, wflag, wflag_ver);
+                                    WfragT32, wflag, wflag_ver, de_max);
+  if (de_max) return fail(ctx, NG_ERR_INVALID, "mp_win_bwd_edge: only the sixteen-wave kernel writes de_max");
   MpWinEdgeArgs a{};
   a.N = N; a.K = K; a.ntiles = cdiv(N, WTA);
   const int64_t per = win_tiles_per_wg(a.ntiles, ctx->num_cu, 8);
@@ -837,10 +838,15 @@
 
 bool mp_win_bwd_enabled(int F, int E, int K) { return mp_win_bwd_supported(F, E, K) && !sw().mp_layered; }
 
+bool mp_win_bwd_de_max_ok(const ng_ctx* ctx, int64_t N, int K, int F, int E) {
+  return mp_win_bwd_enabled(F, E, K) && mp_win_bwd_h2() && sw().mp_w16 && mp_win16_bwd_edge_supported(E, K) &&
+         mp_win16_bwd_edge_de_max_ok(ctx, N);
+}
+
 int mp_win_bwd(ng_ctx* ctx, hipStream_t st, int64_t N, int K, int E, int act, const float* h, const int32_t* nlist,
                const float* e, const float* inv_degree, const float* w, const float* s_save, const int32_t* csc_ptr,
                const int32_t* csc_edge, const float* dh_out, float* dh_in, float* de, int de_accum, float* dw,
-               const float* csc_rec) {
+               const float* csc_rec, float* de_max) {
   const int KF = E * WF;
   const size_t dw_scr = dw ? mp_win_node_scratch_floats(ctx, E) : 0;
   const bool h2 = mp_win_bwd_h2();
@@ -883,7 +889,7 @@
   if (rc) return rc;
   const unsigned wver = pack_flag_version(ctx);
   rc = mp_win_bwd_edge(ctx, st, N, K, E, act, h, nlist, inv_degree, WfragT, s_save, dh_out, dP, de, de_accum, dummy, guard,
-                       WfragT32, wflag, wver);
+                       WfragT32, wflag, wver, de_max);
   if (rc) return rc;
   if (!csc_rec) {
     rc = mp_win_records(ctx, st, N, K, E, csc_ptr, csc_edge, e, rec);
diff --git a/nmrgnn_amd/csrc/ng_internal.h b/nmrgnn_amd/csrc/ng_internal.h
--- a/nmrgnn_amd/csrc/ng_internal.h
+++ b/nmrgnn_amd/csrc/ng_internal.h
@@ -137,10 +137,12 @@
             const float* e, float* A);
 PackJob mpw_bwd_job(int E, const float* w, float* outT, float* outN, float* f32T, float* f32N, unsigned* flag, RangeGuard guard);
 bool mp_win16_bwd_edge_supported(int E, int K);
+constexpr int DE_ABSMAX_LEN = NG_DE_ABSMAX_LEN;
+bool mp_win16_bwd_edge_de_max_ok(const ng_ctx* ctx, int64_t N);
 int mp_win16_bwd_edge_launch(ng_ctx* ctx, hipStream_t st, int64_t N, int K, int E, int act, const float* h, const int32_t* nlist,
                              const float* inv_degree, const float* WfragT, const float* s_save, const float* dh_out, float* dP,
                              float* de, int de_accum, float* dummy, RangeGuard guard, const float* WfragT32, const unsigned* wflag,
-                             unsigned wflag_ver);
+                             unsigned wflag_ver, float* de_max = nullptr);
 bool mp_win16_supported(int E, int K);
 int mp_win16_launch(ng_ctx* ctx, hipStream_t st, int64_t N, int K, int E, int act, int residual, const float* h,
                     const int32_t* nlist, const float* e, const float* inv_degree, const float* Wfrag, const float* Wf32,
@@ -157,7 +159,7 @@
 int mp_win_bwd_edge(ng_ctx* ctx, hipStream_t st, int64_t N, int K, int E, int act, const float* h,
                     const int32_t* nlist, const float* inv_degree, const float* WfragT, const float* s_save,
                     const float* dh_out, float* dP, float* de, int de_accum, float* dummy, RangeGuard guard,
-                    const float* WfragT32, const unsigned* wflag = nullptr, unsigned wflag_ver = 0);
+                    const float* WfragT32, const unsigned* wflag = nullptr, unsigned wflag_ver = 0, float* de_max = nullptr);
 
 int mp_win_records(ng_ctx* ctx, hipStream_t st, int64_t N, int K, int E, const int32_t* csc_ptr,
                    const int32_t* csc_edge, const float* e, float* rec, const int32_t* row_of = nullptr, int64_t n_entries = 0);
@@ -170,10 +172,11 @@
                     const unsigned* wflag = nullptr, unsigned wflag_ver = 0);
 
 bool mp_win_bwd_enabled(int F, int E, int K);
+bool mp_win_bwd_de_max_ok(const ng_ctx* ctx, int64_t N, int K, int F, int E);
 int mp_win_bwd(ng_ctx* ctx, hipStream_t st, int64_t N, int K, int E, int act, const float* h, const int32_t* nlist,
                const float* e, const float* inv_degree, const float* w, const float* s_save, const int32_t* csc_ptr,
                const int32_t* csc_edge, const float* dh_out, float* dh_in, float* de, int de_accum, float* dw,
-               const float* csc_rec);
+               const float* csc_rec, float* de_max = nullptr);
 
 bool head_fast_supported(int Fh, int C);
 int head_loss_graphs_per_wg(ng_ctx* ctx, int G, int Fh, int C, int64_t max_graph_atoms);
diff --git a/nmrgnn_amd/csrc/node_ops.hip b/nmrgnn_amd/csrc/node_ops.hip
--- a/nmrgnn_amd/csrc/node_ops.hip
+++ b/nmrgnn_amd/csrc/node_ops.hip
@@ -628,28 +628,43 @@
   }
 }
 
-__global__ void add_noise_live_kernel(uint64_t seed, uint64_t offset, int64_t n, const float* __restrict__ x,
-                                      const float* __restrict__ y, float alpha, const int32_t* __restrict__ pos,
-                                      float* __restrict__ out_c, const uint64_t* __restrict__ staged) {
+__global__ __launch_bounds__(256) void add_noise_live_kernel(uint64_t seed, uint64_t offset, int64_t n, const float* __restrict__ x,
+                                                             const float* __restrict__ y, float alpha, const int32_t* __restrict__ pos,
+                                                             float* __restrict__ out_c, const uint64_t* __restrict__ staged) {
+  __shared__ __attribute__((aligned(16))) float sz[1024];
   if (staged) seed = staged[0];
   const int64_t n4 = (n + 3) / 4;
-  for (int64_t q = (int64_t)blockIdx.x * blockDim.x + threadIdx.x; q < n4;
-       q += (int64_t)gridDim.x * blockDim.x) {
-    float z[4];
-    if (y) {
-      for (int k = 0; k < 4; ++k) z[k] = q * 4 + k < n ? y[q * 4 + k] : 0.f;
-    } else {
-      uint32_t r[4];
-      philox4x32(seed, offset + (uint64_t)q, r);
-      const float r0 = sqrtf(-2.0f * logf(u01(r[0]))), t0 = 6.28318530717958648f * u01(r[1]);
-      const float r1 = sqrtf(-2.0f * logf(u01(r[2]))), t1 = 6.28318530717958648f * u01(r[3]);
-      z[0] = r0 * cosf(t0); z[1] = r0 * sinf(t0); z[2] = r1 * cosf(t1); z[3] = r1 * sinf(t1);
-    }
+  const int tid = threadIdx.x;
+  for (int64_t qb = (int64_t)blockIdx.x * 256; qb < n4; qb += (int64_t)gridDim.x * 256) {
+    const int64_t g0 = qb * 4 + tid;
+    int32_t pv[4];
+    float xv[4], zv[4];
+#pragma unroll
+    for (int k = 0; k < 4; ++k) {
+      const int64_t g = g0 + 256 * k;
+      pv[k] = g < n ? pos[g] : -1;
+      xv[k] = g < n ? x[g] : 0.f;
+      zv[k] = (y && g < n) ? y[g] : 0.f;
+    }
+    if (!y) {
+      const int64_t q = qb + tid;
+      float z[4] = {0.f, 0.f, 0.f, 0.f};
+      if (q < n4) {
+        uint32_t r[4];
+        philox4x32(seed, offset + (uint64_t)q, r);
+        const float r0 = sqrtf(-2.0f * logf(u01(r[0]))), t0 = 6.28318530717958648f * u01(r[1]);
+        const float r1 = sqrtf(-2.0f * logf(u01(r[2]))), t1 = 6.28318530717958648f * u01(r[3]);
+        z[0] = r0 * cosf(t0); z[1] = r0 * sinf(t0); z[2] = r1 * cosf(t1); z[3] = r1 * sinf(t1);
+      }
+      __syncthreads();
+      *reinterpret_cast<float4*>(sz + 4 * tid) = make_float4(z[0], z[1], z[2], z[3]);
+      __syncthreads();
+#pragma unroll
+      for (int k = 0; k < 4; ++k) zv[k] = sz[256 * k + tid];
+    }
+#pragma unroll
     for (int k = 0; k < 4; ++k)
-      if (q * 4 + k < n) {
-        const int32_t p = pos[q * 4 + k];
-        if (p >= 0) out_c[p] = x[q * 4 + k] + alpha * z[k];
-      }
+      if (pv[k] >= 0) out_c[pv[k]] = xv[k] + alpha * zv[k];
   }
 }
 
@@ -832,15 +847,30 @@
                                    const float* s_save, const int32_t* csc_ptr, const int32_t* csc_edge,
                                    const float* dh_out, float* dh_in, float* de, int de_accum,
                                    float* dw, const float* csc_rec) {
+  return ng_mp_layer_bwd_rec_max(ctx, stream, N, K, F, E, act, h, nlist, e, inv_degree, w, A_save, s_save, csc_ptr, csc_edge,
+                                 dh_out, dh_in, de, de_accum, dw, csc_rec, nullptr);
+}
+
+extern "C" int ng_mp_layer_bwd_de_max_ok(ng_ctx* ctx, int64_t N, int K, int F, int E) {
+  return ctx && mp_win_bwd_de_max_ok(ctx, N, K, F, E) ? 1 : 0;
+}
+
+extern "C" int ng_mp_layer_bwd_rec_max(ng_ctx* ctx, void* stream, int64_t N, int K, int F, int E, int act,
+                                       const float* h, const int32_t* nlist, const float* e,
+                                       const float* inv_degree, const float* w, const float* A_save,
+                                       const float* s_save, const int32_t* csc_ptr, const int32_t* csc_edge,
+                                       const float* dh_out, float* dh_in, float* de, int de_accum,
+                                       float* dw, const float* csc_rec, float* de_absmax) {
   if (!ctx) return NG_ERR_INVALID;
   hipStream_t st = (hipStream_t)stream;
+  NG_REQUIRE(ctx, !de_absmax || mp_win_bwd_de_max_ok(ctx, N, K, F, E), "mp_layer_bwd: de_absmax where ng_mp_layer_bwd_de_max_ok says no");
   NG_REQUIRE(ctx, act == NG_ACT_NONE || s_save, "mp_layer_bwd: s_save required for an activation");
   NG_REQUIRE(ctx, F % 4 == 0 && F >= 16 && F <= 256 && (256 % (F / 4)) == 0,
              "mp_layer_bwd: F in {16,32,64,128,256}");
   NG_REQUIRE(ctx, E >= 1 && E <= 64, "mp_layer_bwd: edge_feature_size <= 64");
   if (N > 0 && mp_win_bwd_enabled(F, E, K))
     return mp_win_bwd(ctx, st, N, K, E, act, h, nlist, e, inv_degree, w, s_save, csc_ptr, csc_edge, dh_out, dh_in, de,
-                      de_accum, dw, csc_rec);
+                      de_accum, dw, csc_rec, de_absmax);
   return mp_generic_bwd(ctx, st, N, K, F, E, act, h, nullptr, nlist, nullptr, e, inv_degree, w, A_save, s_save, csc_ptr,
                         csc_edge, dh_out, dh_in, de, de_accum, dw, E <= 3 ? csc_rec : nullptr);
 }
diff --git a/nmrgnn_amd/engine.py b/nmrgnn_amd/engine.py
--- a/nmrgnn_amd/engine.py
+++ b/nmrgnn_amd/engine.py
@@ -315,7 +315,7 @@
                      "ng_edge_mlp_fwd_live")
         return z, z_layout
 
-    def _edge_mlp_bwd(self, n, d_src, d_eff, z, z_layout, de, grads, perm=None, rows=None):
+    def _edge_mlp_bwd(self, n, d_src, d_eff, z, z_layout, de, grads, perm=None, rows=None, de_absmax=None):
         lib, h, st = self.lib, self.ctx.handle, self._st()
         W, _ = self._edge_weights()
         dW, dB = grads
@@ -324,9 +324,10 @@
                                               ptr(self.centers), self.gap, ptr_array(W), ptr(z), ptr(de), ptr_array(dW),
                                               ptr_array(dB), z_layout), "ng_edge_mlp_bwd")
         else:
-            self._ck(lib.ng_edge_mlp_bwd_live(h, st, n, self.H, self.E, self.Le, self.fc_act, ptr(d_src), ptr(d_eff), ptr(perm),
-                                              ptr(rows), ptr(self.centers), self.gap, ptr_array(W), ptr(z), ptr(de),
-                                              ptr_array(dW), ptr_array(dB), z_layout), "ng_edge_mlp_bwd_live")
+            self._ck(lib.ng_edge_mlp_bwd_live_max(h, st, n, self.H, self.E, self.Le, self.fc_act, ptr(d_src), ptr(d_eff), ptr(perm),
+                                                  ptr(rows), ptr(self.centers), self.gap, ptr_array(W), ptr(z), ptr(de),
+                                                  ptr_array(dW), ptr_array(dB), z_layout, ptr(de_absmax)),
+                     "ng_edge_mlp_bwd_live")
 
     def _edge_table_build(self, batch, live, d_eff, tape, training):
         lib, h, st = self.lib, self.ctx.handle, self._st()
@@ -453,6 +454,7 @@
             self._ck(lib.ng_mp_edge_records(h, st, N, K, E, ptr(csc_ptr), ptr(csc_edge), ptr(tp.e), ptr(rec)),
                      "ng_mp_edge_records")
         dh = dx
+        de_absmax = None
         for l in reversed(range(self.L)):
             dhn = self._new(N, F)
             if b.is_csr:
@@ -464,11 +466,13 @@
                          "ng_mp_layer_bwd_csr")
                 dh = dhn
                 continue
-            self._ck(lib.ng_mp_layer_bwd_rec(h, st, N, K, F, E, self.mp_act, ptr(tp.h[l]), ptr(b.nlist_c),
-                                         ptr(tp.e), ptr(b.inv_degree), ptr(P[f"mp/{l}/w"]),
-                                         ptr(tp.A[l]), ptr(tp.S[l]), ptr(csc_ptr), ptr(csc_edge),
-                                         ptr(dh), ptr(dhn), ptr(de), 0 if l == self.L - 1 else 1,
-                                         ptr(wg(f"mp/{l}/w")), ptr(rec)), "ng_mp_layer_bwd")
+            if l == 0 and param_grad and tp.edge_path == "live" and lib.ng_mp_layer_bwd_de_max_ok(h, N, K, F, E):
+                de_absmax = self._new(lib.ng_de_absmax_len())
+            self._ck(lib.ng_mp_layer_bwd_rec_max(h, st, N, K, F, E, self.mp_act, ptr(tp.h[l]), ptr(b.nlist_c),
+                                                 ptr(tp.e), ptr(b.inv_degree), ptr(P[f"mp/{l}/w"]),
+                                                 ptr(tp.A[l]), ptr(tp.S[l]), ptr(csc_ptr), ptr(csc_edge),
+                                                 ptr(dh), ptr(dhn), ptr(de), 0 if l == self.L - 1 else 1,
+                                                 ptr(wg(f"mp/{l}/w")), ptr(rec), ptr(de_absmax)), "ng_mp_layer_bwd")
             dh = dhn
         if not param_grad:
             self._edge_dinput(tp, de, edge_grad)
@@ -483,7 +487,7 @@
             self._edge_mlp_bwd(ne, b.edges, tp.d_eff, tp.z_save, tp.z_layout, de, self._edge_grads())
         elif tp.edge_path == "live":
             perm, _, d_c, n_live = tp.live
-            self._edge_mlp_bwd(ne, d_c, tp.d_eff, tp.z_save, tp.z_layout, de, self._edge_grads(), perm, n_live)
+            self._edge_mlp_bwd(ne, d_c, tp.d_eff, tp.z_save, tp.z_layout, de, self._edge_grads(), perm, n_live, de_absmax)
         elif tp.edge_path == "table_host":
             self._edge_table_backward(tp, de, self._edge_grads())
         else:
```

New measurement: 43.85 million, median of 6. No clear change (+0.3%).
